# raznem/spp-rl

Hardware: AMD Instinct MI355X
Metric: env-steps/sec (rollout+update) SPP-SAC Hopper-v2 (higher is better)
Workload: dtype fp32

## Files before the change

### spp-rl_amd/csrc/api.hip

```cpp
#include <dlfcn.h>
#include <stdarg.h>
#include <stdio.h>
#include <string.h>

#include <algorithm>
#include <memory>
#include <string>
#include <vector>

#include "../../include/spprl.h"
#include "internal.h"
#include "replay.h"
#include "sac_kernels.h"

#include "optim.hip"
#include "ppo.hip"
#include "replay.hip"
#include "stats.hip"
#include "sac.hip"
#include "ddpg.hip"
#include "kset.h"
#ifdef SPP_SINGLE_TU
#include "ks_dw.hip"
#include "ks_sac_hopper.hip"
// ... 507 lines not shown
      else
        hipLaunchKernelGGL(k_st_bracket<kStSampSmall / 1024>, dim3(ob), dim3(1024), 0, st, (const uint32_t*)samp, S,
                           h->sf_bounds, Sl, (int64_t)ob * Sl, 5);
      h->bounds_dp1 = true;
      h->sf_gen = ~0ull;
    }
    StPassArgs pa{h->d, len, h->sf_bounds, pivot, h->sf_part, h->sf_cpart, h->sf_wgl, h->sf_wgn, h->sf_ovf,
                  h->sf_ovf_n, cap, ovf_cap};
    st_launch_pass(pa, nblk, st);
    hipLaunchKernelGGL(k_dp_reduce, dim3(ob, 2), dim3(kStSelThreads), 0, st, ob, nblk, cap, ovf_cap,
                       (const double*)h->sf_part,
                       (const uint32_t*)h->sf_cpart, (const uint32_t*)h->sf_wgl, (const uint32_t*)h->sf_wgn,
                       (const uint32_t*)h->sf_ovf, (const uint32_t*)h->sf_ovf_n, exch, h->dp_cand, dp_ncand);
  } else if (phase <= 5) {
    hipLaunchKernelGGL(k_dp_round, dim3(ob, 2), dim3(kStSelThreads), 0, st, da, phase - 2);
  } else {
    hipLaunchKernelGGL(k_dp_final, dim3(ob, 2), dim3(128), 0, st, da);
  }
  SPP_CHECK_HIP(hipGetLastError());
  return SPP_OK;
}

int sppReplayObsStatsDPHistSize(sppReplayHandle h) {
  if (!h) return -1;
  const int ob = h->d.ob;
  return std::max(ob, std::min(ob, 32) * 4) * 256;
}

sppStatus sppReplayObsStatsDP(sppReplayHandle h, int step, const float* pivot, double* sums, uint32_t* hist,
                              int64_t n_global, float* mean, float* std, float* max_obs, float* min_obs,
                              int first_update, int* done, void* stream) {
  SPP_REQUIRE(h && pivot && sums && hist && mean && std && max_obs && min_obs && done && step >= 0,
              SPP_E_INVALID_ARG, "obs_stats_dp: bad args");
  const int ob = h->d.ob;
  SPP_REQUIRE(ob <= 16 * kStatsColsPerThread, SPP_E_SHAPE, "obs_stats_dp: ob %d > %d", ob, 16 * kStatsColsPerThread);
  SPP_REQUIRE(n_global > 10 && n_global < ((int64_t)1 << 31), SPP_E_INVALID_ARG, "obs_stats_dp: n_global %lld",
              (long long)n_global);
  sppStatus s = stats_alloc(h);
  if (s) return s;
  hipStream_t st = S(stream);
  const int npass = stats_npass(h);
  SPP_REQUIRE(step <= npass + 1, SPP_E_INVALID_ARG, "obs_stats_dp: step %d > %d", step, npass + 1);
  *done = 0;
  if (step == 0) {
    SPP_CHECK_HIP(hipMemsetAsync(hist, 0, sizeof(uint32_t) * sppReplayObsStatsDPHistSize(h), st));
    if (h->len > 0) {
      stats_pass1(h, hist, pivot, st);
      hipLaunchKernelGGL(k_stats_reduce_part, dim3(ob), dim3(256), 0, st, (const double*)h->st_part, kStatsBlocks,
                         ob, sums);
    } else {
      SPP_CHECK_HIP(hipMemsetAsync(sums, 0, sizeof(double) * ob * 2, st));
    }
  } else {
    if (step == 1) {
      hipLaunchKernelGGL(k_stats_sel, dim3(ob), dim3(256), 0, st, hist, 1, ob, 0, ob, 24, 8, 1, (const double*)sums,
                         n_global, h->st_state, h->st_mean, max_obs, min_obs, first_update);
      hipLaunchKernelGGL(k_stats_moments_out, dim3(1), dim3(128), 0, st, h->d, (const double*)h->st_mean, mean, std,
                         pivot);
    } else {
      stats_sel(h, step - 2, hist, n_global, max_obs, min_obs, first_update, st);
    }
    if (step - 1 < npass) {
      if (h->len > 0) stats_pk(h, step - 1, hist, st);
    } else {
      *done = 1;
    }
  }
  SPP_CHECK_HIP(hipGetLastError());
  return SPP_OK;
}

sppStatus sppGaeScan(const float* rew, const float* v, const float* v_next, const uint8_t* done,
                     const uint8_t* end, int64_t T, int64_t E, double gamma, double lam, int mode, float* q_out,
                     float* adv, void* stream) {
  SPP_REQUIRE(T >= 0 && E > 0 && mode >= -1 && mode <= 1, SPP_E_INVALID_ARG, "gae: T=%lld E=%lld mode=%d",
              (long long)T, (long long)E, mode);
  if (T == 0) return SPP_OK;
  SPP_REQUIRE(rew && v && v_next && done && end && adv, SPP_E_INVALID_ARG, "gae: null input");
  if (mode < 0) mode = E >= 64 ? 0 : 1;
  const double disc = lam * gamma;
  if (mode == 0)
    hipLaunchKernelGGL(k_gae_seq, dim3(cdiv(E, 256)), dim3(256), 0, S(stream), rew, v, v_next, done, end, T, E,
                       (float)gamma, disc, q_out, adv);
  else
    hipLaunchKernelGGL(k_gae_scan, dim3(E), dim3(kScanThreads), 0, S(stream), rew, v, v_next, done, end, T, E,
                       (float)gamma, (float)disc, q_out, adv);
  SPP_CHECK_HIP(hipGetLastError());
  return SPP_OK;
}

sppStatus sppPpoClipLoss(const float* lp_old, const float* lp_new, const float* adv, int B, float eps, float* grad,
                         float* out2, void* stream) {
  SPP_REQUIRE(lp_old && lp_new && adv && out2 && B > 0, SPP_E_INVALID_ARG, "clip loss: bad args");
  const int nblk = cdiv(B, 256);
  double* part = nullptr;
  SPP_CHECK_HIP(hipMallocAsync((void**)&part, sizeof(double) * 2 * nblk, S(stream)));
  hipLaunchKernelGGL(k_ppo_clip, dim3(nblk), dim3(256), 0, S(stream), lp_old, lp_new, adv, B, eps, grad, part);
  hipLaunchKernelGGL(k_ppo_clip_finish, dim3(1), dim3(256), 0, S(stream), (const double*)part, nblk, B, out2);
  SPP_CHECK_HIP(hipFreeAsync(part, S(stream)));
  SPP_CHECK_HIP(hipGetLastError());
  return SPP_OK;
}

sppStatus sppAdvNormalize(const float* adv, int64_t n, float* out, void* stream) {
  SPP_REQUIRE(adv && out && n > 0, SPP_E_INVALID_ARG, "adv normalize: bad args");
  const int nblk = (int)std::min<int64_t>(cdiv(n, 256), 1024);
  double* part = nullptr;
  SPP_CHECK_HIP(hipMallocAsync((void**)&part, sizeof(double) * 2 * nblk, S(stream)));
  hipLaunchKernelGGL(k_adv_moments, dim3(nblk), dim3(256), 0, S(stream), adv, n, part);
  hipLaunchKernelGGL(k_adv_norm, dim3(nblk), dim3(256), 0, S(stream), adv, n, (const double*)part, nblk, out);
  SPP_CHECK_HIP(hipFreeAsync(part, S(stream)));
  SPP_CHECK_HIP(hipGetLastError());
  return SPP_OK;
}

sppStatus sppAdvSums(const float* adv, int64_t n, double* sums2, void* stream) {
  SPP_REQUIRE(adv && sums2 && n >= 0, SPP_E_INVALID_ARG, "adv sums: bad args");
  if (n == 0) {
    SPP_CHECK_HIP(hipMemsetAsync(sums2, 0, sizeof(double) * 2, S(stream)));
    return SPP_OK;
  }
  const int nblk = (int)std::min<int64_t>(cdiv(n, 256), 1024);
  double* part = nullptr;
  SPP_CHECK_HIP(hipMallocAsync((void**)&part, sizeof(double) * 2 * nblk, S(stream)));
  hipLaunchKernelGGL(k_adv_moments, dim3(nblk), dim3(256), 0, S(stream), adv, n, part);
  hipLaunchKernelGGL(k_adv_sum2, dim3(1), dim3(64), 0, S(stream), (const double*)part, nblk, sums2);
  SPP_CHECK_HIP(hipFreeAsync(part, S(stream)));
  SPP_CHECK_HIP(hipGetLastError());
  return SPP_OK;
}

sppStatus sppAdvNormalizeGlobal(const float* adv, int64_t n_local, const double* sums2, int64_t n_global, float* out,
                                void* stream) {
  SPP_REQUIRE(adv && out && sums2 && n_local >= 0 && n_global > 0, SPP_E_INVALID_ARG, "adv normalize dp: bad args");
  if (n_local == 0) return SPP_OK;
  hipLaunchKernelGGL(k_adv_norm_g, dim3((int)std::min<int64_t>(cdiv(n_local, 256), 1024)), dim3(256), 0, S(stream),
                     adv, n_local, sums2, n_global, out);
  SPP_CHECK_HIP(hipGetLastError());
  return SPP_OK;
}

sppStatus sppSynthEnvStep(const float* A, const float* obs, const float* action, int E, int ob, int ac,
                          float* next_obs, float* reward, void* stream) {
  SPP_REQUIRE(A && obs && action && next_obs && reward && E > 0, SPP_E_INVALID_ARG, "synth env: bad args");
  hipLaunchKernelGGL(k_synth_env, dim3(cdiv((int64_t)E * ob, 256)), dim3(256), 0, S(stream), A, obs, action, E, ob, ac, next_obs,
                     reward);
  SPP_CHECK_HIP(hipGetLastError());
  return SPP_OK;
}


sppStatus sppRandUniform(float* out, int64_t n, const float* lo, const float* hi, int period, uint64_t seed,
                         uint64_t offset, void* stream) {
  SPP_REQUIRE((out || n == 0) && lo && hi && period > 0, SPP_E_INVALID_ARG, "rand uniform: bad args");
  if (n == 0) return SPP_OK;
  hipLaunchKernelGGL(k_rand_uniform, dim3(cdiv((n + 3) / 4, 256)), dim3(256), 0, S(stream), out, n, lo, hi, period,
                     seed, offset);
  SPP_CHECK_HIP(hipGetLastError());
  return SPP_OK;
}

sppStatus sppEpisodeAccum(const float* rew, const uint8_t* end, int E, float* ep_ret, double* sums, void* stream) {
  SPP_REQUIRE(rew && ep_ret && sums && E > 0, SPP_E_INVALID_ARG, "episode accum: bad args");
  hipLaunchKernelGGL(k_episode_accum, dim3(cdiv(E, 256)), dim3(256), 0, S(stream), rew, end, E, ep_ret, sums);
  SPP_CHECK_HIP(hipGetLastError());
  return SPP_OK;
}

sppStatus sppSynthEnvReset(float* obs, const uint8_t* mask, int E, int ob, uint64_t seed, uint64_t offset,
                           void* stream) {
  SPP_REQUIRE(obs && E > 0 && ob > 0, SPP_E_INVALID_ARG, "synth reset: bad args");
  hipLaunchKernelGGL(k_synth_reset, dim3(cdiv((int64_t)E * ob, 256)), dim3(256), 0, S(stream), obs, mask, E, ob, seed,
                     offset);
  SPP_CHECK_HIP(hipGetLastError());
  return SPP_OK;
}

sppStatus sppObsNormalize(const float* x, int64_t rows, int ob, const float* lo, const float* hi, const float* mean,
                          const float* std, int min_max, int inverse, float* out, void* stream) {
  SPP_REQUIRE(x && out && rows >= 0 && ob > 0, SPP_E_INVALID_ARG, "normalize: bad args");
  SPP_REQUIRE(min_max ? (lo && hi) : (mean && std), SPP_E_INVALID_ARG, "normalize: missing statistics");
  if (rows == 0) return SPP_OK;
  const int64_t n = rows * ob;
  hipLaunchKernelGGL(k_obs_normalize, dim3(cdiv(n, 256)), dim3(256), 0, S(stream), x, n, ob, lo, hi, mean, std,
                     min_max, inverse, out);
  SPP_CHECK_HIP(hipGetLastError());
  return SPP_OK;
}
}

namespace spp {

struct NetBufs {
  float *p = nullptr, *g = nullptr, *m = nullptr, *v = nullptr;
  int64_t n = 0;
};

template <typename T>
struct DevArray {
  T* ptr = nullptr;
  size_t n = 0;
  hipError_t alloc(size_t count) {
    n = count;
    return hipMalloc(&ptr, sizeof(T) * std::max<size_t>(count, 1));
  }
  void release() {
    if (ptr) hipFree(ptr);
    ptr = nullptr;
  }
};

struct DwSet {
  DevArray<float> slab;
  DevArray<DwJob> jobs;
  DevArray<int> items;
  int B = -1;
  int j0[2] = {0, 0}, nj[2] = {0, 0}, ioff[2] = {0, 0}, nitems[2] = {0, 0};
  int nlds[2] = {0, 0};
  int64_t max_elems[2] = {1, 1};
  bool bf16 = false;
  void release() { slab.release(); jobs.release(); items.release(); }
};

static bool find_kset(int algo, int ob, int aout, int ac, bool acmc, bool bf16, KernelSet* ks) {
  if (bf16) {
#if !defined(SPP_ONLY_HOPPER) || defined(SPP_ONLY_BF16)
    return algo == SPP_ALGO_SAC_ACM && kset_sac_bf16(ob, aout, ac, acmc, ks);
#else
    return false;
#endif
  }
  if (algo == SPP_ALGO_SAC) {
#ifndef SPP_ONLY_HOPPER
    return kset_sac_vanilla(ob, aout, ac, acmc, ks);
#else
    return false;
#endif
  }
  if (algo == SPP_ALGO_DDPG) {
#ifndef SPP_ONLY_HOPPER
    return kset_ddpg_vanilla(ob, aout, ac, acmc, ks);
#else
    return false;
#endif
  }
  if (algo == SPP_ALGO_SAC_ACM) {
    if (kset_sac_hopper(ob, aout, ac, acmc, ks)) return true;
#if defined(SPP_ONLY_HOPPER) && defined(SPP_WITH_HCHEETAH)
    if (kset_sac_hcheetah(ob, aout, ac, acmc, ks)) return true;
#endif
#ifndef SPP_ONLY_HOPPER
    if (kset_sac_hcheetah(ob, aout, ac, acmc, ks)) return true;
    if (kset_sac_ant(ob, aout, ac, acmc, ks)) return true;
    if (kset_sac_small(ob, aout, ac, acmc, ks)) return true;
  } else if (algo == SPP_ALGO_DDPG_ACM) {
    if (kset_ddpg(ob, aout, ac, acmc, ks)) return true;
    if (kset_ddpg_ant(ob, aout, ac, acmc, ks)) return true;
#endif
  }
  return false;
}

}

struct sppAgent {
  sppAgentConfig cfg{};
  int device = 0, num_cu = 256;
  bool team_ok = true;
  KernelSet ks{};
  NetBufs net[SPP_NET_COUNT];
  int64_t nsize[SPP_NET_COUNT] = {};
  int cin = 0, Bmax = 0, Bpmax = 0;
  int64_t steps[4] = {0, 0, 0, 0};
  const float *lo = nullptr, *hi = nullptr, *mean = nullptr, *std = nullptr;
  double* alpha_state = nullptr;
  float* alpha_f32 = nullptr;
  DevArray<float> limits;
  DevArray<float4> pk;
  std::vector<PackJob> pj_actor, pj_acm, pj_targ, pj_critic_fwd, pj_critic_all, pj_acmreg;
  bool ddpg = false;
  bool plain = false;
  DevArray<PackJob> d_pj;
  int o_actor = 0, o_acm = 0, o_targ = 0, o_cfwd = 0, o_call = 0, o_acmreg = 0;
  std::vector<TabSeg> tab;
  int tab_floats = 0;
  ActorDev actor{};
  CriticDev critic[2]{}, targ[2]{};
  AcmDev acm{};
  const float4* acm_W1n = nullptr;
  BAcmDev bacm{};
  ActorDev actor_targ{};
  const float4 *bacm_W1n = nullptr, *bacm_W21n = nullptr;
  BAcmScratch bz{};
  float *RBH = nullptr, *RBH1 = nullptr, *RS21 = nullptr, *RBP1 = nullptr, *RPZ = nullptr, *RPZ21 = nullptr;
  DevArray<float> scratch;
  float *S = nullptr, *S2 = nullptr, *ACT = nullptr, *AENV = nullptr, *R = nullptr, *DN = nullptr, *EPS1 = nullptr,
        *EPS2 = nullptr;
  float *H1[2] = {}, *H2[2] = {}, *D1[2] = {}, *D2[2] = {}, *DQ[2] = {};
  float *AH1 = nullptr, *AH2 = nullptr, *AD1 = nullptr, *AD2 = nullptr, *ADH = nullptr;
  float *Z1 = nullptr, *Z2 = nullptr, *T3 = nullptr, *part = nullptr;
  float *aux = nullptr;
  float* GAD = nullptr;
  uint64_t* MASK = nullptr;
  float *RX = nullptr, *RZ1 = nullptr, *RZ2 = nullptr, *RP1 = nullptr, *RP2 = nullptr, *RP3 = nullptr;
  DwSet dws[2];
  DevArray<AdamJob> d_adam;
  int cur_B = -1;
  float* w3p[2] = {};
  int64_t w3p_stride = 0;
  float* alpha_grad = nullptr;
  DevArray<float> sgd_slab;
  DevArray<int> sgd_sync;
  int sgd_max_wg = -1;
  bool timing = false;
  std::vector<hipEvent_t> tev[5];
  size_t tused[5] = {0, 0, 0, 0, 0};
};

static void tmark(sppAgent* a, int kind, hipStream_t st) {
  if (!a->timing) return;
  auto& v = a->tev[kind];
  if (a->tused[kind] == v.size()) {
    hipEvent_t e;
    hipEventCreate(&e);
    v.push_back(e);
  }
  hipEventRecord(v[a->tused[kind]++], st);
}

namespace spp {

static int64_t sac_actor_size(int ob, int aout) { return 256LL * ob + 256 + 65536 + 256 + 2LL * (aout * 256 + aout); }
static int64_t critic_size(int cin) { return 256LL * cin + 256 + 65536 + 256 + 256 + 1; }
static int64_t acm_size(int in, int ac) { return 64LL * in + 64 + 32 * 64 + 32 + (int64_t)ac * 32 + ac; }
static int64_t ddpg_actor_size(int ob, int aout) { return 256LL * ob + 256 + 65536 + 256 + (int64_t)aout * 256 + aout; }
static int64_t bacm_size(int in, int ac) {
  return 1 + ac + 100LL * in + 100 + 50 * 100 + 50 + 50LL * in + 50 + (int64_t)ac * 50 + ac;
}

static MapDesc nat(int n) { return MapDesc{MAP_NAT, n, 0, 0, 0}; }
static MapDesc cat(int n0, int n1) { return MapDesc{MAP_CAT, n0, blocks_of(n0), n1, n0}; }
static MapDesc pair(int n) { return MapDesc{MAP_PAIR, n, 0, 0, 0}; }

}

static sppStatus build_packs(sppAgent* a) {
  const int ob = a->cfg.ob, aout = a->cfg.aout, ac = a->cfg.ac;
  const int ca = a->cfg.acm_critic ? ac : aout;
  const int cin = ob + ca;
  for (int k = 0; k < SPP_NET_COUNT; ++k) {
    const bool used = a->ddpg ? (k == SPP_NET_ACTOR || k == SPP_NET_CRITIC1 || k == SPP_NET_CRITIC1_TARG ||
                                 (k == SPP_NET_ACM && !a->plain) || k == SPP_NET_ACTOR_TARG)
                              : k != SPP_NET_ACTOR_TARG;
    SPP_REQUIRE(!used || a->net[k].p, SPP_E_STATE, "network %d parameters not bound", k);
  }
  struct MatSpec {
    std::vector<PackJob>* list;
    PackJob job;
    const float4** slot;
  };
  std::vector<MatSpec> ms;
  auto M = [&](std::vector<PackJob>* list, const float* W, const float* W2, int split, int ld, int trans, int coff,
               MapDesc out, MapDesc in, int NBO, int NBI, const float4** slot, int ib = 0) {
    PackJob j{W, W2, split, ld, trans, coff, out, in, NBO, NBI, ib, nullptr, a->cfg.mlp_bf16 ? 1 : 0};
    ms.push_back({list, j, slot});
  };
  a->tab.clear();
  int toff = 0;
  auto T = [&](const float* v, int n, const float* v2 = nullptr, int n2 = 0) {
    const int off = toff, tot = (int)round_up(n + n2, 32);
    a->tab.push_back(TabSeg{v, n, v2 ? n : tot, off, 0});
    if (v2) a->tab.push_back(TabSeg{v2, n2, tot - n, off + n, 0});
    toff += tot;
    return off;
  };
  if (!a->ddpg) {
    {
      const float* P = a->net[SPP_NET_ACTOR].p;
      const float *W1 = P, *b1 = W1 + 256 * ob, *W2 = b1 + 256, *b2 = W2 + 65536, *Wp = b2 + 256, *bp = Wp + aout * 256,
                  *Ws = bp + aout, *bs = Ws + aout * 256;
      M(&a->pj_actor, W1, nullptr, 1 << 30, ob, 0, 0, nat(256), nat(ob), 8, blocks_of(ob), &a->actor.W1);
      M(&a->pj_actor, W2, nullptr, 1 << 30, 256, 0, 0, nat(256), nat(256), 8, 8, &a->actor.W2, 1);
      M(&a->pj_actor, Wp, Ws, aout, 256, 0, 0, nat(2 * aout), nat(256), blocks_of(2 * aout), 8, &a->actor.Wh, 1);
      M(&a->pj_actor, W2, nullptr, 1 << 30, 256, 1, 0, nat(256), nat(256), 8, 8, &a->actor.W2T, 1);
      M(&a->pj_actor, Wp, Ws, aout, 256, 1, 0, nat(256), pair(aout), 8, (aout + 15) / 16, &a->actor.WhT);
      if (a->cfg.mlp_bf16)
        M(&a->pj_actor, Wp, Ws, aout, 256, 0, 0, pair(aout), nat(256), (aout + 15) / 16, 8, &a->actor.WhP, 1);
      a->actor.tb1 = T(b1, 256);
      a->actor.tb2 = T(b2, 256);
      a->actor.tbh = T(bp, aout, bs, aout);
    }
  } else {
    for (int t = 0; t < 2; ++t) {
      const float* P = a->net[t == 0 ? SPP_NET_ACTOR : SPP_NET_ACTOR_TARG].p;
      ActorDev& ad = t == 0 ? a->actor : a->actor_targ;
      std::vector<PackJob>* l = t == 0 ? &a->pj_actor : &a->pj_targ;
      const float *W1 = P, *b1 = W1 + 256 * ob, *W2 = b1 + 256, *b2 = W2 + 65536, *W3 = b2 + 256, *b3 = W3 + aout * 256;
      M(l, W1, nullptr, 1 << 30, ob, 0, 0, nat(256), nat(ob), 8, blocks_of(ob), &ad.W1);
      M(l, W2, nullptr, 1 << 30, 256, 0, 0, nat(256), nat(256), 8, 8, &ad.W2, 1);
      M(l, W3, nullptr, 1 << 30, 256, 0, 0, nat(aout), nat(256), blocks_of(aout), 8, &ad.Wh, 1);
      if (t == 0) {
        M(l, W2, nullptr, 1 << 30, 256, 1, 0, nat(256), nat(256), 8, 8, &ad.W2T, 1);
        M(l, W3, nullptr, 1 << 30, 256, 1, 0, nat(256), nat(aout), 8, blocks_of(aout), &ad.WhT);
      }
      ad.tb1 = T(b1, 256);
      ad.tb2 = T(b2, 256);
      ad.tbh = T(b3, aout);
    }
  }
  if (!a->ddpg) {
    {
      const float* P = a->net[SPP_NET_ACM].p;
      const int in = 2 * ob;
      const float *W1 = P, *b1 = W1 + 64 * in, *W2 = b1 + 64, *b2 = W2 + 32 * 64, *W3 = b2 + 32, *b3 = W3 + ac * 32;
      M(&a->pj_acm, W1, nullptr, 1 << 30, in, 0, 0, nat(64), cat(ob, aout), 2, blocks_of(ob) + blocks_of(aout),
        &a->acm.W1);
      M(&a->pj_acm, W2, nullptr, 1 << 30, 64, 0, 0, nat(32), nat(64), 1, 2, &a->acm.W2);
      M(&a->pj_acm, W3, nullptr, 1 << 30, 32, 0, 0, nat(ac), nat(32), 1, 1, &a->acm.W3);
      M(&a->pj_acm, W3, nullptr, 1 << 30, 32, 1, 0, nat(32), nat(ac), 1, 1, &a->acm.W3T);
      M(&a->pj_acm, W2, nullptr, 1 << 30, 64, 1, 0, nat(64), nat(32), 2, 1, &a->acm.W2T);
      M(&a->pj_acm, W1, nullptr, 1 << 30, in, 1, ob, nat(aout), nat(64), blocks_of(aout), 2, &a->acm.W1Ta);
      M(&a->pj_acm, W1, nullptr, 1 << 30, in, 0, 0, nat(64), nat(in), 2, blocks_of(in), &a->acm_W1n);
      a->acm.tb1 = T(b1, 64);
      a->acm.tb2 = T(b2, 32);
      a->acm.tb3 = T(b3, ac);
    }
  } else if (!a->plain) {
    const float* P = a->net[SPP_NET_ACM].p;
    const int in = 2 * ob;
    const float *t = P, *t1 = P + 1, *W1 = t1 + ac, *b1 = W1 + 100 * in, *W2 = b1 + 100, *b2 = W2 + 50 * 100,
                *W21 = b2 + 50, *b21 = W21 + 50 * in, *W3 = b21 + 50, *b3 = W3 + ac * 50;
    BAcmDev& B = a->bacm;
    const int nbi = blocks_of(ob) + blocks_of(aout);
    M(&a->pj_acm, W1, nullptr, 1 << 30, in, 0, 0, nat(100), cat(ob, aout), 4, nbi, &B.W1);
    M(&a->pj_acm, W21, nullptr, 1 << 30, in, 0, 0, nat(50), cat(ob, aout), 2, nbi, &B.W21);
    M(&a->pj_acm, W2, nullptr, 1 << 30, 100, 0, 0, nat(50), nat(100), 2, 4, &B.W2);
    M(&a->pj_acm, W3, nullptr, 1 << 30, 50, 0, 0, nat(ac), nat(50), 1, 2, &B.W3);
    M(&a->pj_acm, W3, nullptr, 1 << 30, 50, 1, 0, nat(50), nat(ac), 2, 1, &B.W3T);
    M(&a->pj_acm, W2, nullptr, 1 << 30, 100, 1, 0, nat(100), nat(50), 4, 2, &B.W2T);
    M(&a->pj_acm, W1, nullptr, 1 << 30, in, 1, ob, nat(aout), nat(100), blocks_of(aout), 4, &B.W1Ta);
    M(&a->pj_acm, W21, nullptr, 1 << 30, in, 1, ob, nat(aout), nat(50), blocks_of(aout), 2, &B.W21Ta);
    M(&a->pj_acm, W1, nullptr, 1 << 30, in, 0, 0, nat(100), nat(in), 4, blocks_of(in), &a->bacm_W1n);
    M(&a->pj_acm, W21, nullptr, 1 << 30, in, 0, 0, nat(50), nat(in), 2, blocks_of(in), &a->bacm_W21n);
    B.tb1 = T(b1, 100);
    B.tb21 = T(b21, 50);
    B.tb2 = T(b2, 50);
    B.tb3 = T(b3, ac);
    B.t = t;
    B.t1 = t1;
  }
  for (int t = 0; t < 4; ++t) {
    if (a->ddpg && (t == 1 || t == 3)) continue;
    const int netid = t < 2 ? SPP_NET_CRITIC1 + t : SPP_NET_CRITIC1_TARG + (t - 2);
    CriticDev& cd = t < 2 ? a->critic[t] : a->targ[t - 2];
    const float* P = a->net[netid].p;
    const float *W1 = P, *b1 = W1 + 256 * cin, *W2 = b1 + 256, *b2 = W2 + 65536, *w3 = b2 + 256, *b3 = w3 + 256;
    std::vector<PackJob>* fl = t < 2 ? &a->pj_critic_fwd : &a->pj_targ;
    M(fl, W1, nullptr, 1 << 30, cin, 0, 0, nat(256), cat(ob, ca), 8, blocks_of(ob) + blocks_of(ca), &cd.W1);
    M(fl, W2, nullptr, 1 << 30, 256, 0, 0, nat(256), nat(256), 8, 8, &cd.W2, 1);
    if (t < 2) {
      M(fl, W2, nullptr, 1 << 30, 256, 1, 0, nat(256), nat(256), 8, 8, &cd.W2T, 1);
      M(fl, W1, nullptr, 1 << 30, cin, 1, ob, nat(ca), nat(256), blocks_of(ca), 8, &cd.W1Ta, 1);
    }
    cd.tb1 = T(b1, 256);
    cd.tb2 = T(b2, 256);
    cd.tw3 = T(w3, 256);
    cd.b3 = b3;
  }
  a->tab_floats = toff;
  const int extra = 3 * (int)round_up(aout, 32) + (int)round_up(std::max(ac, 1), 32);
  SPP_REQUIRE(toff + extra <= kTabMax && (int)a->tab.size() + 4 <= kTabSegs, SPP_E_SHAPE,
              "LDS table too large (%d floats, %d segments)", toff + extra, (int)a->tab.size() + 4);
  size_t nf4 = 0;
  for (auto& m : ms) nf4 += (size_t)m.job.NBO * m.job.NBI * 4 * 64;
  a->pk.release();
  SPP_CHECK_HIP(a->pk.alloc(nf4));
  size_t of = 0;
  for (auto& m : ms) {
    m.job.dst = a->pk.ptr + of;
    *m.slot = m.job.dst;
    of += (size_t)m.job.NBO * m.job.NBI * 4 * 64;
    m.list->push_back(m.job);
  }
  a->pj_critic_all = a->pj_critic_fwd;
  std::vector<PackJob> all;
  a->o_actor = (int)all.size(); all.insert(all.end(), a->pj_actor.begin(), a->pj_actor.end());
  a->o_acm = (int)all.size(); all.insert(all.end(), a->pj_acm.begin(), a->pj_acm.end());
  a->o_targ = (int)all.size(); all.insert(all.end(), a->pj_targ.begin(), a->pj_targ.end());
  a->o_cfwd = (int)all.size(); all.insert(all.end(), a->pj_critic_fwd.begin(), a->pj_critic_fwd.end());
  a->d_pj.release();
  SPP_CHECK_HIP(a->d_pj.alloc(all.size()));
  SPP_CHECK_HIP(hipMemcpy(a->d_pj.ptr, all.data(), sizeof(PackJob) * all.size(), hipMemcpyHostToDevice));
  return SPP_OK;
}

static void launch_pack(sppAgent* a, int off, int n, hipStream_t st) {
  if (n > 0) hipLaunchKernelGGL(k_pack_matrix, dim3(64, n), dim3(256), 0, st, (const PackJob*)(a->d_pj.ptr + off));
}

#ifndef SPP_DW_BIG16
#define SPP_DW_BIG16 1
#endif
static sppStatus finalize_dw(DwSet& D, std::vector<DwJob>& jobs, int nph, int Bp, int B, int num_cu) {
  auto is_big = [](const DwJob& j) {
    return (int64_t)round_up(j.N, 32) * round_up(j.K0 + j.K1, 32) >= 128 * 128;
  };
  auto lds_big = [Bp](const DwJob& j) {
    return Bp >= 8192 && j.N == 256 && j.K0 == 256 && j.K1 == 0 &&
           (!j.bf16 || (SPP_DW_BIG16 && j.a_bf && j.x_bf && Bp % 64 == 0));
  };
  auto assign_splits = [&](int first, int count) {
    double big[2] = {0.0, 0.0};
    for (int i = first; i < first + count; ++i)
      if (!jobs[i].fused && is_big(jobs[i]))
        big[lds_big(jobs[i]) ? 0 : 1] += (double)round_up(jobs[i].N, 32) * round_up(jobs[i].K0 + jobs[i].K1, 32);
    for (int i = first; i < first + count; ++i) {
      DwJob& j = jobs[i];
      if (j.fused) continue;
      const double pm = (double)round_up(j.N, 32) * round_up(j.K0 + j.K1, 32);
      const bool thin_n = j.N <= 128, thin_k = j.K0 + j.K1 <= 128;
      j.wsplit = thin_n && thin_k ? 4 : (thin_n != thin_k ? 2 : 1);
      int ns = is_big(j) ? (int)std::lround(num_cu * pm / big[lds_big(j) ? 0 : 1])
                         : std::min(cdiv(Bp, 2048), std::max(1, 256 / j.wsplit));
      if (!is_big(j)) ns = std::max(ns, std::min(cdiv(Bp, 32 * j.wsplit), 4));
      ns = std::max(1, std::min(ns, std::max(1, Bp / 32)));
      j.split_len = (int)round_up(cdiv(Bp, ns), lds_big(j) && j.bf16 ? 64 : 32 * j.wsplit);
      j.nsplit = cdiv(Bp, j.split_len);
    }
  };
  for (int ph = 0; ph < nph; ++ph) assign_splits(D.j0[ph], D.nj[ph]);
  size_t need = 0;
  for (int ph = 0; ph < nph; ++ph) {
    size_t off = 0;
    for (int j = D.j0[ph]; j < D.j0[ph] + D.nj[ph]; ++j) {
      if (jobs[j].nsplit * jobs[j].wsplit > 1) {
        jobs[j].slab = nullptr;
        off += (size_t)jobs[j].nsplit * jobs[j].wsplit * jobs[j].slab_stride;
      }
    }
    need = std::max(need, off);
  }
  if (need > D.slab.n) {
    D.slab.release();
    SPP_CHECK_HIP(D.slab.alloc(need));
  }
  std::vector<int> items;
  for (int ph = 0; ph < nph; ++ph) {
    size_t off = 0;
    std::vector<int> jj, ss;
    for (int j = D.j0[ph]; j < D.j0[ph] + D.nj[ph]; ++j) {
      if (jobs[j].nsplit * jobs[j].wsplit > 1) {
        jobs[j].slab = D.slab.ptr + off;
        off += (size_t)jobs[j].nsplit * jobs[j].wsplit * jobs[j].slab_stride;
      }
    }
    D.nlds[ph] = 0;
    for (int pass = 0; pass < 3; ++pass)
      for (int j = D.j0[ph]; j < D.j0[ph] + D.nj[ph]; ++j) {
        const int cls = lds_big(jobs[j]) ? 0 : (is_big(jobs[j]) ? 1 : 2);
        if (cls != pass || jobs[j].fused) continue;
        for (int sp = 0; sp < jobs[j].nsplit; ++sp) {
          jj.push_back(j - D.j0[ph]);
          ss.push_back(sp);
          if (pass == 0) ++D.nlds[ph];
        }
      }
    D.max_elems[ph] = 1;
    for (int j = D.j0[ph]; j < D.j0[ph] + D.nj[ph]; ++j) {
      const int64_t el = (int64_t)jobs[j].N * (jobs[j].K0 + jobs[j].K1) + jobs[j].N;
      D.max_elems[ph] = std::max<int64_t>(D.max_elems[ph], el * dw_red_group(jobs[j].nsplit * jobs[j].wsplit, el));
    }
    D.ioff[ph] = (int)items.size();
    D.nitems[ph] = (int)jj.size();
    items.insert(items.end(), jj.begin(), jj.end());
    items.insert(items.end(), ss.begin(), ss.end());
  }
  D.jobs.release();
  D.items.release();
  SPP_CHECK_HIP(D.jobs.alloc(jobs.size()));
  SPP_CHECK_HIP(D.items.alloc(items.size()));
  SPP_CHECK_HIP(hipMemcpy(D.jobs.ptr, jobs.data(), sizeof(DwJob) * jobs.size(), hipMemcpyHostToDevice));
  SPP_CHECK_HIP(hipMemcpy(D.items.ptr, items.data(), sizeof(int) * items.size(), hipMemcpyHostToDevice));
  D.B = B;
  D.bf16 = !jobs.empty() && jobs[0].bf16;
  for (const DwJob& j : jobs)
    if ((j.bf16 != 0) != D.bf16) return SPP_E_STATE;
  return SPP_OK;
}

static int phase_grid(sppAgent* a, int Bp);
static int sac_grid(sppAgent* a, int Bp);
static int sac_critic_grid(sppAgent* a, int Bp);
static bool sac_team(sppAgent* a, int Bp);
static bool ddpg_team(sppAgent* a, int Bp);
static int ddpg_grid(sppAgent* a, int Bp);
static sppStatus build_dw(sppAgent* a, int set, int B) {
  const int Bp = (int)round_up(B, 32);
  const int ob = a->cfg.ob, aout = a->cfg.aout, ac = a->cfg.ac;
  const int ca = a->cfg.acm_critic ? ac : aout, cin = ob + ca;
  std::vector<DwJob> jobs;
  std::vector<const float*> b16;
  if (a->cfg.mlp_bf16 && !a->ddpg && set == 0)
    b16 = {a->H1[0], a->H1[1], a->H2[0], a->H2[1], a->D1[0], a->D1[1], a->D2[0], a->D2[1],
           a->AH1, a->AH2, a->AD1, a->AD2};
  auto is16 = [&](const float* p) { return p && std::find(b16.begin(), b16.end(), p) != b16.end(); };
  auto J = [&](const float* A, int N, const float* X0, int K0, const float* X1, int K1, float* dW, float* db,
               int nrow2 = -1, float* dW2 = nullptr, float* db2 = nullptr) {
    DwJob j{};
    j.A = A; j.N = N; j.X0 = X0; j.K0 = K0; j.X1 = X1; j.K1 = K1; j.dW = dW; j.db = db; j.Bp = Bp;
    j.nrow2 = nrow2 < 0 ? N : nrow2;
    j.dW2 = dW2; j.db2 = db2;
    j.slab_stride = round_up((int64_t)N * (K0 + K1) + N, 4);
    j.bf16 = a->cfg.mlp_bf16 ? 1 : 0;
    j.a_bf = is16(A) ? 1 : 0;
    j.x_bf = is16(X0) ? 1 : 0;
    jobs.push_back(j);
  };
  DwSet& D = a->dws[set];
  int nph = 0;
  if (a->ddpg) {
    if (set == 0) {
      float* G = a->net[SPP_NET_CRITIC1].g;
      float *gW1 = G, *gb1 = gW1 + 256 * cin, *gW2 = gb1 + 256, *gb2 = gW2 + 65536, *gw3 = gb2 + 256, *gb3 = gw3 + 256;
      J(a->D1[0], 256, a->S, ob, a->cfg.acm_critic ? a->AENV : a->ACT, ca, gW1, gb1);
      J(a->D2[0], 256, a->H1[0], 256, nullptr, 0, gW2, gb2);
      int fused0 = -1;
      if (ob <= 32) {
        J(nullptr, 1, nullptr, 256, nullptr, 0, gw3, gb3);
        jobs.back().fused = 1;
        jobs.back().nsplit = ddpg_grid(a, Bp) * (ddpg_team(a, Bp) ? kTeamDCritic : kWavesPerWG);
        jobs.back().wsplit = 1;
        fused0 = (int)jobs.size() - 1;
      } else {
        J(a->DQ[0], 1, a->H2[0], 256, nullptr, 0, gw3, gb3);
      }
      D.j0[0] = 0;
      D.nj[0] = (int)jobs.size();
      float* A = a->net[SPP_NET_ACTOR].g;
      float *aW1 = A, *ab1 = aW1 + 256 * ob, *aW2 = ab1 + 256, *ab2 = aW2 + 65536, *aW3 = ab2 + 256,
            *ab3 = aW3 + aout * 256;
      J(a->AD1, 256, a->S, ob, nullptr, 0, aW1, ab1);
      J(a->AD2, 256, a->AH1, 256, nullptr, 0, aW2, ab2);
      J(a->ADH, aout, a->AH2, 256, nullptr, 0, aW3, ab3);
      D.j0[1] = D.nj[0];
      D.nj[1] = (int)jobs.size() - D.nj[0];
      nph = 2;
      sppStatus s = finalize_dw(D, jobs, nph, Bp, B, a->num_cu);
      a->w3p[0] = a->w3p[1] = fused0 >= 0 ? jobs[fused0].slab : nullptr;
      a->w3p_stride = fused0 >= 0 ? jobs[fused0].slab_stride : 0;
      return s;
    } else {
      SPP_REQUIRE(!a->plain, SPP_E_STATE, "vanilla DDPG has no ACM to regress");
      float* G = a->net[SPP_NET_ACM].g;
      const int in = 2 * ob;
      float *gW1 = G + 1 + ac, *gb1 = gW1 + 100 * in, *gW2 = gb1 + 100, *gb2 = gW2 + 50 * 100, *gW21 = gb2 + 50,
            *gb21 = gW21 + 50 * in, *gW3 = gb21 + 50, *gb3 = gW3 + ac * 50;
      J(a->RBP1, 100, a->RX, in, nullptr, 0, gW1, gb1);
      J(a->RPZ, 50, a->RBH, 100, nullptr, 0, gW2, gb2);
      J(a->RPZ21, 50, a->RX, in, nullptr, 0, gW21, gb21);
      J(a->RP3, ac, a->RBH1, 50, nullptr, 0, gW3, gb3);
      D.j0[0] = 0;
      D.nj[0] = (int)jobs.size();
      nph = 1;
    }
  } else if (set == 0) {
    const bool fuse3 = !a->cfg.mlp_bf16 || SPP_BF16_FUSE3;
    int fused_idx[2] = {-1, -1};
    for (int i = 0; i < 2; ++i) {
      float* G = a->net[SPP_NET_CRITIC1 + i].g;
      float *gW1 = G, *gb1 = gW1 + 256 * cin, *gW2 = gb1 + 256, *gb2 = gW2 + 65536, *gw3 = gb2 + 256, *gb3 = gw3 + 256;
      J(a->D1[i], 256, a->S, ob, a->cfg.acm_critic ? a->AENV : a->ACT, ca, gW1, gb1);
      J(a->D2[i], 256, a->H1[i], 256, nullptr, 0, gW2, gb2);
      if (!fuse3) {
        J(a->DQ[i], 1, a->H2[i], 256, nullptr, 0, gw3, gb3);
        continue;
      }
      J(nullptr, 1, nullptr, 256, nullptr, 0, gw3, gb3);
      jobs.back().fused = 1;
      jobs.back().nsplit = sac_critic_grid(a, Bp) * (sac_team(a, Bp) ? kTeamCritic : kWavesPerWG);
      jobs.back().wsplit = 1;
      fused_idx[i] = (int)jobs.size() - 1;
    }
    D.j0[0] = 0;
    D.nj[0] = (int)jobs.size();
    float* G = a->net[SPP_NET_ACTOR].g;
    float *gW1 = G, *gb1 = gW1 + 256 * ob, *gW2 = gb1 + 256, *gb2 = gW2 + 65536, *gWp = gb2 + 256,
          *gbp = gWp + aout * 256, *gWs = gbp + aout, *gbs = gWs + aout * 256;
    J(a->AD1, 256, a->S, ob, nullptr, 0, gW1, gb1);
    J(a->AD2, 256, a->AH1, 256, nullptr, 0, gW2, gb2);
    J(a->ADH, 2 * aout, a->AH2, 256, nullptr, 0, gWp, gbp, aout, gWs, gbs);
    D.j0[1] = D.nj[0];
    D.nj[1] = (int)jobs.size() - D.nj[0];
    nph = 2;
    sppStatus s = finalize_dw(D, jobs, nph, Bp, B, a->num_cu);
    for (int i = 0; i < 2; ++i) a->w3p[i] = fuse3 ? jobs[fused_idx[i]].slab : nullptr;
    a->w3p_stride = fuse3 ? jobs[fused_idx[0]].slab_stride : 0;
    return s;
  } else {
    float* G = a->net[SPP_NET_ACM].g;
    const int in = 2 * ob;
    float *gW1 = G, *gb1 = gW1 + 64 * in, *gW2 = gb1 + 64, *gb2 = gW2 + 32 * 64, *gW3 = gb2 + 32, *gb3 = gW3 + ac * 32;
    J(a->RP1, 64, a->RX, in, nullptr, 0, gW1, gb1);
    J(a->RP2, 32, a->RZ1, 64, nullptr, 0, gW2, gb2);
    J(a->RP3, ac, a->RZ2, 32, nullptr, 0, gW3, gb3);
    D.j0[0] = 0;
    D.nj[0] = (int)jobs.size();
    nph = 1;
  }
  return finalize_dw(D, jobs, nph, Bp, B, a->num_cu);
}


static void launch_dw_set(DwSet& D, int ph, hipStream_t st) {
  const int* ij = D.items.ptr + D.ioff[ph];
  const int* is = ij + D.nitems[ph];
  const DwJob* jobs = D.jobs.ptr + D.j0[ph];
  launch_dw_kernels(jobs, ij, is, D.nitems[ph], D.nlds[ph], D.nj[ph], D.max_elems[ph], D.bf16, st);
}
static void launch_dw(sppAgent* a, int set, int ph, hipStream_t st) { launch_dw_set(a->dws[set], ph, st); }

static sppStatus build_adam(sppAgent* a) {
  AdamJob jobs[4] = {};
  for (int i = 0; i < (a->ddpg ? 1 : 2); ++i) {
    NetBufs& n = a->net[SPP_NET_CRITIC1 + i];
    jobs[i] = AdamJob{n.p, n.g, n.m, n.v, a->net[SPP_NET_CRITIC1_TARG + i].p, n.n};
  }
  NetBufs& na = a->net[SPP_NET_ACTOR];
  jobs[2] = AdamJob{na.p, na.g, na.m, na.v, a->ddpg ? a->net[SPP_NET_ACTOR_TARG].p : nullptr, na.n};
  NetBufs& nm = a->net[SPP_NET_ACM];
  jobs[3] = AdamJob{nm.p, nm.g, nm.m, nm.v, nullptr, nm.n};
  if (!a->d_adam.ptr) SPP_CHECK_HIP(a->d_adam.alloc(4));
  SPP_CHECK_HIP(hipMemcpy(a->d_adam.ptr, jobs, sizeof(jobs), hipMemcpyHostToDevice));
  return SPP_OK;
}

static void launch_adam(sppAgent* a, int first, int count, int64_t n, int64_t step, float lr, float tau,
                        hipStream_t st) {
  const double bc1 = 1.0 - std::pow(0.9, (double)step), bc2s = std::sqrt(1.0 - std::pow(0.999, (double)step));
  hipLaunchKernelGGL(k_adam, dim3(std::max(1, std::min(cdiv(n, 256 * 4), 1024)), count), dim3(256), 0, st,
                     (const AdamJob*)(a->d_adam.ptr + first), (float)(-(lr / bc1)), (float)bc2s, tau);
}

static SacArgs make_args(sppAgent* a, int B) {
  SacArgs p{};
  p.B = B;
  p.Bp = (int)round_up(B, 32);
  p.inv_B = 1.f / (float)B;
  p.S = a->S; p.S2 = a->S2; p.ACT = a->ACT; p.AENV = a->AENV; p.R = a->R; p.DN = a->DN;
  p.EPS1 = a->EPS1; p.EPS2 = a->EPS2;
  p.min_max = a->cfg.min_max_denormalize;
  p.lo = a->lo; p.hi = a->hi; p.mean = a->mean; p.std = a->std;
  p.actor_lim = a->limits.ptr;
  p.acm_lim = a->limits.ptr + a->cfg.aout;
  p.gamma = a->cfg.gamma;
  p.custom_loss = a->cfg.custom_loss;
  p.norm_closs = a->cfg.norm_closs;
  p.alpha = a->alpha_f32;
  p.actor = a->actor;
  for (int i = 0; i < 2; ++i) {
    p.critic[i] = a->critic[i];
    p.targ[i] = a->targ[i];
    p.H1[i] = a->H1[i]; p.H2[i] = a->H2[i]; p.D1[i] = a->D1[i]; p.D2[i] = a->D2[i]; p.DQ[i] = a->DQ[i];
    p.W3P[i] = a->w3p[i];
  }
  p.w3p_stride = a->w3p_stride;
  p.acm = a->acm;
  p.bacm = a->bacm;
  p.actor_targ = a->actor_targ;
  p.AH1 = a->AH1; p.AH2 = a->AH2; p.AD1 = a->AD1; p.AD2 = a->AD2; p.ADH = a->ADH;
  p.part = a->part;
  p.nseg = (int)a->tab.size();
  for (int i = 0; i < p.nseg; ++i) p.seg[i] = a->tab[i];
  int off = a->tab_floats;
  auto X = [&](const float* v, int n) {
    const int o = off, np = (int)round_up(std::max(n, 1), 32);
    p.seg[p.nseg++] = TabSeg{v ? v : a->limits.ptr, v ? n : 0, np, o, 0};
    off += np;
    return o;
  };
  const int aout = a->cfg.aout;
  p.t_lim = X(a->limits.ptr, aout);
  p.t_alim = X(a->limits.ptr + aout, a->cfg.ac);
  p.t_n0 = X(p.min_max ? a->lo : a->mean, aout);
  p.t_n1 = X(p.min_max ? a->hi : a->std, aout);
  return p;
}

static int phase_grid(sppAgent* a, int Bp) {
  const int ntiles = Bp / 32;
  return std::max(1, std::min(cdiv(ntiles, kWavesPerWG), a->num_cu));
}
static bool sac_team(sppAgent* a, int Bp) {
  return a->ks.critic_team && a->ks.actor_team && a->team_ok && Bp / 32 <= a->num_cu;
}
static int sac_grid(sppAgent* a, int Bp) {
  return sac_team(a, Bp) ? std::max(1, std::min(Bp / 32, a->num_cu)) : phase_grid(a, Bp);
}
static int sac_critic_grid(sppAgent* a, int Bp) {
  const int nt = std::max(1, Bp / 32);
  return sac_team(a, Bp) && 2 * nt <= a->num_cu ? 2 * nt : sac_grid(a, Bp);
}

static bool ddpg_team(sppAgent* a, int Bp) {
  return a->ks.dcritic_team && a->ks.dactor_team && a->team_ok && Bp / 32 <= a->num_cu;
}
static int ddpg_grid(sppAgent* a, int Bp) {
  return ddpg_team(a, Bp) ? std::max(1, std::min(Bp / 32, a->num_cu)) : phase_grid(a, Bp);
}

static sppStatus check_ready(sppAgent* a) {
  SPP_REQUIRE(a->ddpg || (a->alpha_state && a->alpha_f32), SPP_E_STATE, "alpha not bound");
  SPP_REQUIRE(a->cfg.min_max_denormalize ? (a->lo && a->hi) : (a->mean && a->std), SPP_E_STATE,
              "normalizer not bound");
  SPP_REQUIRE(a->limits.ptr, SPP_E_STATE, "limits not set");
  if (!a->pk.ptr) {
    sppStatus s = build_packs(a);
    if (s) return s;
    if ((s = build_adam(a))) return s;
    a->dws[0].B = a->dws[1].B = -1;
  }
  return SPP_OK;
}

extern "C" {

sppStatus sppAgentCreate(sppAgentHandle* out, const sppAgentConfig* cfg, int device) {
  SPP_REQUIRE(out && cfg, SPP_E_INVALID_ARG, "null arg");
  SPP_REQUIRE(cfg->algo == SPP_ALGO_SAC_ACM || cfg->algo == SPP_ALGO_DDPG_ACM || cfg->algo == SPP_ALGO_SAC ||
                  cfg->algo == SPP_ALGO_DDPG,
              SPP_E_INVALID_ARG, "unsupported algo %d", cfg->algo);
  SPP_REQUIRE(cfg->algo != SPP_ALGO_SAC || (cfg->acm_critic == 0 && cfg->aout == cfg->ac && cfg->custom_loss == 0.f),
              SPP_E_INVALID_ARG, "vanilla SAC: the actor emits the env action (aout == ac), no ACM critic / loss");
  SPP_REQUIRE(cfg->algo != SPP_ALGO_DDPG || (cfg->acm_critic == 0 && cfg->aout == cfg->ac && cfg->custom_loss == 0.f),
              SPP_E_INVALID_ARG, "vanilla DDPG: the actor emits the env action (aout == ac), no ACM critic / loss");
  SPP_REQUIRE(cfg->algo != SPP_ALGO_DDPG || cfg->mlp_bf16 == 0, SPP_E_INVALID_ARG, "vanilla DDPG: fp32 only");
  SPP_REQUIRE(cfg->max_batch > 0, SPP_E_INVALID_ARG, "max_batch must be > 0");
  KernelSet ks;
  SPP_REQUIRE(find_kset(cfg->algo, cfg->ob, cfg->aout, cfg->ac, cfg->acm_critic != 0, cfg->mlp_bf16 != 0, &ks),
              SPP_E_SHAPE, "no kernel instantiation for algo %d (ob=%d, aout=%d, ac=%d, bf16=%d)", cfg->algo, cfg->ob,
              cfg->aout, cfg->ac, cfg->mlp_bf16);
  SPP_CHECK_HIP(hipSetDevice(device));
  auto a = std::make_unique<sppAgent>();
  a->cfg = *cfg;
  a->device = device;
  a->ks = ks;
  hipDeviceProp_t prop;
  SPP_CHECK_HIP(hipGetDeviceProperties(&prop, device));
  a->num_cu = prop.multiProcessorCount;
  {
    const char* t = getenv("SPP_SAC_TEAM");
    a->team_ok = !(t && t[0] == '0');
  }
  const int ob = cfg->ob, aout = cfg->aout, ac = cfg->ac;
  a->cin = ob + (cfg->acm_critic ? ac : aout);
  a->ddpg = cfg->algo == SPP_ALGO_DDPG_ACM || cfg->algo == SPP_ALGO_DDPG;
  a->plain = cfg->algo == SPP_ALGO_SAC || cfg->algo == SPP_ALGO_DDPG;
  const bool dd = a->ddpg;
  a->nsize[SPP_NET_ACTOR] = dd ? ddpg_actor_size(ob, aout) : sac_actor_size(ob, aout);
  a->nsize[SPP_NET_ACTOR_TARG] = dd ? ddpg_actor_size(ob, aout) : 0;
  a->nsize[SPP_NET_CRITIC1] = a->nsize[SPP_NET_CRITIC1_TARG] = critic_size(a->cin);
  a->nsize[SPP_NET_CRITIC2] = a->nsize[SPP_NET_CRITIC2_TARG] = dd ? 0 : critic_size(a->cin);
  a->nsize[SPP_NET_ACM] = dd ? (a->plain ? 0 : bacm_size(2 * ob, ac)) : acm_size(2 * ob, ac);
  a->Bmax = cfg->max_batch;
  const int64_t Bp = round_up(cfg->max_batch, 32);
  SPP_REQUIRE((int64_t)Bp * 256 * 4 < ((int64_t)1 << 31), SPP_E_SHAPE, "max_batch %d too large (31-bit buffer offsets)",
              cfg->max_batch);
  a->Bpmax = (int)Bp;
  const int64_t ntiles = Bp / 32;
  const int64_t per = Bp;
  int64_t total = 0;
  auto take = [&](int64_t rows) { int64_t o = total; total += rows * per; return o; };
  const int64_t oS = take(ob), oS2 = take(ob), oACT = take(aout), oAENV = take(ac), oR = take(1), oDN = take(1),
                oE1 = take(aout), oE2 = take(aout);
  int64_t oH1[2] = {}, oH2[2] = {}, oD1[2] = {}, oD2[2] = {}, oDQ[2] = {};
  for (int i = 0; i < (dd ? 1 : 2); ++i) {
    oH1[i] = take(256); oH2[i] = take(256); oD1[i] = take(256); oD2[i] = take(256); oDQ[i] = take(1);
  }
  const int64_t oAH1 = take(256), oAH2 = take(256), oAD1 = take(256), oAD2 = take(256), oADH = take(2 * aout);
  const int64_t oZ1 = take(dd ? 128 : 64), oZ2 = take(dd ? 64 : 32), oT3 = take(ac);
  const int64_t oRX = take(2 * ob), oRZ1 = take(dd ? 128 : 64), oRZ2 = take(dd ? 64 : 32), oRP1 = take(dd ? 128 : 64),
                oRP2 = take(dd ? 64 : 32), oRP3 = take(ac);
  const int64_t oRS21 = dd ? take(64) : 0, oRPZ21 = dd ? take(64) : 0;
  const int64_t oGAD = take(aout), oMASK = take(16);
  const int64_t oPart = total;
  total += ntiles * kBParts + 64;
  const int64_t oAux = total;
  total += 16;
  hipError_t e = a->scratch.alloc(total);
  if (e != hipSuccess) {
    set_error("scratch alloc %.2f GB: %s", total * 4.0 / 1e9, hipGetErrorString(e));
    return SPP_E_OOM;
  }
  SPP_CHECK_HIP(hipMemset(a->scratch.ptr, 0, sizeof(float) * total));
  float* b = a->scratch.ptr;
  a->S = b + oS; a->S2 = b + oS2; a->ACT = b + oACT; a->AENV = b + oAENV; a->R = b + oR; a->DN = b + oDN;
  a->EPS1 = b + oE1; a->EPS2 = b + oE2;
  for (int i = 0; i < 2; ++i) {
    a->H1[i] = b + oH1[i]; a->H2[i] = b + oH2[i]; a->D1[i] = b + oD1[i]; a->D2[i] = b + oD2[i]; a->DQ[i] = b + oDQ[i];
  }
  a->AH1 = b + oAH1; a->AH2 = b + oAH2; a->AD1 = b + oAD1; a->AD2 = b + oAD2; a->ADH = b + oADH;
  a->Z1 = b + oZ1; a->Z2 = b + oZ2; a->T3 = b + oT3;
  a->GAD = b + oGAD;
  a->MASK = reinterpret_cast<uint64_t*>(b + oMASK);
  a->RX = b + oRX; a->RZ1 = b + oRZ1; a->RZ2 = b + oRZ2; a->RP1 = b + oRP1; a->RP2 = b + oRP2; a->RP3 = b + oRP3;
  if (dd) {
    a->bz = BAcmScratch{a->Z1, a->Z2, a->T3};
    a->RBH = a->RZ1; a->RBH1 = a->RZ2; a->RBP1 = a->RP1; a->RPZ = a->RP2;
    a->RS21 = b + oRS21; a->RPZ21 = b + oRPZ21;
  }
  a->part = b + oPart;
  a->aux = b + oAux;
  SPP_CHECK_HIP(a->limits.alloc(aout + ac));
  *out = a.release();
  return SPP_OK;
}

sppStatus sppAgentDestroy(sppAgentHandle a) {
  if (!a) return SPP_OK;
  hipSetDevice(a->device);
  hipDeviceSynchronize();
  a->limits.release(); a->pk.release(); a->d_pj.release();
  for (auto& v : a->tev)
    for (auto e : v) hipEventDestroy(e);
  a->scratch.release(); a->d_adam.release();
  for (auto& D : a->dws) D.release();
  delete a;
  return SPP_OK;
}

sppStatus sppAgentNetSize(sppAgentHandle a, int net, int64_t* n) {
  SPP_REQUIRE(a && n && net >= 0 && net < SPP_NET_COUNT, SPP_E_INVALID_ARG, "bad net id");
  *n = a->nsize[net];
  return SPP_OK;
}

sppStatus sppAgentBindNet(sppAgentHandle a, int net, float* p, float* g, float* m, float* v) {
  SPP_REQUIRE(a && net >= 0 && net < SPP_NET_COUNT && p, SPP_E_INVALID_ARG, "bind: bad args");
  const bool trainable = net == SPP_NET_ACTOR || net == SPP_NET_CRITIC1 || net == SPP_NET_CRITIC2 || net == SPP_NET_ACM;
  SPP_REQUIRE(!trainable || (g && m && v), SPP_E_INVALID_ARG, "bind: trainable net %d needs grad/m/v", net);
  const bool changed = a->net[net].p != p || a->net[net].g != g;
  a->net[net] = NetBufs{p, g, m, v, a->nsize[net]};
  if (changed) {
    a->pk.release();
    a->pj_actor.clear(); a->pj_acm.clear(); a->pj_targ.clear(); a->pj_critic_fwd.clear(); a->pj_critic_all.clear();
    a->tab.clear();
  }
  return SPP_OK;
}

sppStatus sppAgentSetLimits(sppAgentHandle a, const float* actor_lim, const float* acm_lim) {
  SPP_REQUIRE(a && actor_lim && acm_lim, SPP_E_INVALID_ARG, "null");
  SPP_CHECK_HIP(hipMemcpy(a->limits.ptr, actor_lim, sizeof(float) * a->cfg.aout, hipMemcpyHostToDevice));
  SPP_CHECK_HIP(hipMemcpy(a->limits.ptr + a->cfg.aout, acm_lim, sizeof(float) * a->cfg.ac, hipMemcpyHostToDevice));
  return SPP_OK;
}

sppStatus sppAgentBindNormalizer(sppAgentHandle a, const float* lo, const float* hi, const float* mean,
                                 const float* std) {
  SPP_REQUIRE(a, SPP_E_INVALID_ARG, "null");
  a->lo = lo; a->hi = hi; a->mean = mean; a->std = std;
  return SPP_OK;
}

sppStatus sppAgentBindAlpha(sppAgentHandle a, double* st, float* af) {
  SPP_REQUIRE(a && st && af, SPP_E_INVALID_ARG, "null");
  a->alpha_state = st;
  a->alpha_f32 = af;
  return SPP_OK;
}

sppStatus sppAgentSetLr(sppAgentHandle a, float actor_lr, float critic_lr, float alpha_lr, float acm_lr) {
  SPP_REQUIRE(a, SPP_E_INVALID_ARG, "null handle");
  if (actor_lr >= 0.f) a->cfg.actor_lr = actor_lr;
  if (critic_lr >= 0.f) a->cfg.critic_lr = critic_lr;
  if (alpha_lr >= 0.f) a->cfg.alpha_lr = alpha_lr;
  if (acm_lr >= 0.f) a->cfg.acm_lr = acm_lr;
  return SPP_OK;
}
sppStatus sppAgentSetSteps(sppAgentHandle a, int64_t s0, int64_t s1, int64_t s2, int64_t s3) {
  SPP_REQUIRE(a, SPP_E_INVALID_ARG, "null");
  a->steps[0] = s0; a->steps[1] = s1; a->steps[2] = s2; a->steps[3] = s3;
  return SPP_OK;
}
sppStatus sppAgentGetSteps(sppAgentHandle a, int64_t* s) {
  SPP_REQUIRE(a && s, SPP_E_INVALID_ARG, "null");
  for (int i = 0; i < 4; ++i) s[i] = a->steps[i];
  return SPP_OK;
}

static sppStatus stage(sppAgentHandle a, const sppBatch* bt, const float* e1, const float* e2, hipStream_t st) {
  SPP_REQUIRE(bt && bt->B > 0 && bt->B <= a->Bmax, SPP_E_SHAPE, "batch B=%d outside (0, max_batch=%d]",
              bt ? bt->B : -1, a->Bmax);
  SPP_REQUIRE(bt->obs && bt->next_obs && bt->reward && bt->done && bt->acm_action, SPP_E_INVALID_ARG,
              "batch: null field");
  SPP_REQUIRE(a->cfg.acm_critic || bt->action, SPP_E_INVALID_ARG, "batch.action required without acm_critic");
  StageArgs s{};
  s.B = bt->B; s.Bp = (int)round_up(bt->B, 32); s.ob = a->cfg.ob; s.aout = a->cfg.aout; s.ac = a->cfg.ac;
  s.obs = bt->obs; s.next_obs = bt->next_obs; s.act = bt->action; s.rew = bt->reward; s.acm = bt->acm_action;
  s.done = bt->done; s.eps1 = e1; s.eps2 = e2;
  s.S = a->S; s.S2 = a->S2; s.ACT = a->ACT; s.AENV = a->AENV; s.R = a->R; s.DN = a->DN; s.EPS1 = a->EPS1;
  s.EPS2 = a->EPS2;
  hipLaunchKernelGGL(k_stage_batch, dim3(cdiv(s.Bp, 256)), dim3(256), 0, st, s);
  a->cur_B = bt->B;
  return SPP_OK;
}

static sppStatus critic_grads_staged(sppAgentHandle a, float* losses, hipStream_t st) {
  SPP_REQUIRE(!a->ddpg, SPP_E_STATE, "not a SAC_AcM agent");
  const int B = a->cur_B;
  SPP_REQUIRE(B > 0, SPP_E_STATE, "no staged batch");
  sppStatus s = check_ready(a);
  if (s) return s;
  if (a->dws[0].B != B) {
    s = build_dw(a, 0, B);
    if (s) return s;
  }
  launch_pack(a, a->o_actor, (int)(a->pj_actor.size() + a->pj_acm.size() + a->pj_targ.size() + a->pj_critic_fwd.size()),
              st);
  SacArgs p = make_args(a, B);
  const int grid = sac_critic_grid(a, p.Bp);
  tmark(a, 0, st);
  const bool team = sac_team(a, p.Bp);
  hipLaunchKernelGGL(team ? a->ks.critic_team : a->ks.critic, dim3(grid), dim3(team ? 64 * kTeamCritic : 256), 0, st, p);
  tmark(a, 0, st);
  SPP_CHECK_HIP(hipGetLastError());
  tmark(a, 2, st);
  launch_dw(a, 0, 0, st);
  tmark(a, 2, st);
  hipLaunchKernelGGL(k_finalize_critic, dim3(1), dim3(kFinThreads), 0, st, (const float*)a->part, p.Bp / 32, B, losses);
  SPP_CHECK_HIP(hipGetLastError());
  return SPP_OK;
}

sppStatus sppSacAcmCriticGrads(sppAgentHandle a, const sppBatch* bt, const float* eps_next, float* losses,
                               void* stream) {
  SPP_REQUIRE(a, SPP_E_INVALID_ARG, "null");
  if (bt) {
    sppStatus s = stage(a, bt, eps_next, nullptr, S(stream));
    if (s) return s;
  } else if (eps_next) {
    const int Bp = (int)round_up(a->cur_B, 32);
    SPP_REQUIRE(a->cur_B > 0, SPP_E_STATE, "no staged batch");
    hipLaunchKernelGGL(k_eps_copy_fm, dim3(cdiv((int64_t)a->cfg.aout * Bp, 256)), dim3(256), 0, S(stream), eps_next,
                       a->EPS1, a->cfg.aout, a->cur_B, Bp);
  }
  return critic_grads_staged(a, losses, S(stream));
}

sppStatus sppSacAcmCriticApply(sppAgentHandle a, void* stream) {
  SPP_REQUIRE(a && a->d_adam.ptr, SPP_E_STATE, "agent not ready");
  a->steps[1] += 1;
  tmark(a, 3, S(stream));
  launch_adam(a, 0, 2, a->net[SPP_NET_CRITIC1].n, a->steps[1], a->cfg.critic_lr, a->cfg.tau, S(stream));
  tmark(a, 3, S(stream));
  SPP_CHECK_HIP(hipGetLastError());
  return SPP_OK;
}

static sppStatus actor_grads(sppAgentHandle a, float* losses, hipStream_t st) {
  SPP_REQUIRE(!a->ddpg, SPP_E_STATE, "not a SAC_AcM agent");
  const int B = a->cur_B;
  SPP_REQUIRE(B > 0, SPP_E_STATE, "no staged batch");
  launch_pack(a, a->o_cfwd, (int)a->pj_critic_fwd.size(), st);
  SacArgs p = make_args(a, B);
  AcmScratch z{a->Z1, a->Z2, a->T3, a->GAD, a->MASK};
  const int grid = sac_grid(a, p.Bp);
  tmark(a, 1, st);
  const bool team = sac_team(a, p.Bp);
  hipLaunchKernelGGL(team ? a->ks.actor_team : a->ks.actor, dim3(grid), dim3(team ? 64 * kTeamActor : 256), 0, st, p, z);
  if (a->ks.actor_heads) hipLaunchKernelGGL(a->ks.actor_heads, dim3(grid), dim3(256), 0, st, p, z);
  tmark(a, 1, st);
  SPP_CHECK_HIP(hipGetLastError());
  tmark(a, 2, st);
  launch_dw(a, 0, 1, st);
  tmark(a, 2, st);
  hipLaunchKernelGGL(k_actor_partials, dim3(1), dim3(kFinThreads), 0, st, (const float*)a->part, p.Bp / 32, B, a->cfg.aout,
                     a->cfg.custom_loss, (double)a->cfg.target_entropy, a->alpha_grad ? a->alpha_grad : a->aux,
                     losses);
  SPP_CHECK_HIP(hipGetLastError());
  return SPP_OK;
}

sppStatus sppSacAcmActorGrads(sppAgentHandle a, const float* eps_cur, float* losses, void* stream) {
  SPP_REQUIRE(a, SPP_E_INVALID_ARG, "null");
  const int B = a->cur_B;
  SPP_REQUIRE(B > 0, SPP_E_STATE, "no staged batch");
  const int Bp = (int)round_up(B, 32);
  if (eps_cur)
    hipLaunchKernelGGL(k_eps_copy_fm, dim3(cdiv((int64_t)a->cfg.aout * Bp, 256)), dim3(256), 0, S(stream), eps_cur,
                       a->EPS2, a->cfg.aout, B, Bp);
  return actor_grads(a, losses, S(stream));
}

sppStatus sppAgentBindAlphaGrad(sppAgentHandle a, float* g) {
  SPP_REQUIRE(a, SPP_E_INVALID_ARG, "null");
  a->alpha_grad = g;
  return SPP_OK;
}

sppStatus sppSacAcmDrawEps(sppAgentHandle a, uint64_t seed, uint64_t counter, void* stream) {
  SPP_REQUIRE(a && a->cur_B > 0, SPP_E_STATE, "no staged batch");
  const int B = a->cur_B, Bp = (int)round_up(B, 32);
  SPP_REQUIRE((int64_t)a->cfg.aout * Bp < ((int64_t)1 << 31), SPP_E_SHAPE, "draw_eps: aout * Bp >= 2^31");
  const int64_t quads = (int64_t)a->cfg.aout * Bp / 4;
  hipLaunchKernelGGL(k_eps_fm, dim3(cdiv(quads, 256), 2), dim3(256), 0, S(stream), a->EPS1, a->cfg.aout, B, Bp, seed,
                     2 * counter, a->EPS2, 2 * counter + 1);
  SPP_CHECK_HIP(hipGetLastError());
  return SPP_OK;
}

sppStatus sppAgentReadEps(sppAgentHandle a, int which, float* out, void* stream) {
  SPP_REQUIRE(a && out && (which == 0 || which == 1), SPP_E_INVALID_ARG, "read_eps: bad args");
  SPP_REQUIRE(a->cur_B > 0, SPP_E_STATE, "no staged batch");
  const int B = a->cur_B, Bp = (int)round_up(B, 32);
  hipLaunchKernelGGL(k_eps_read_fm, dim3(cdiv((int64_t)a->cfg.aout * B, 256)), dim3(256), 0, S(stream),
                     (const float*)(which ? a->EPS2 : a->EPS1), out, a->cfg.aout, B, Bp);
  SPP_CHECK_HIP(hipGetLastError());
  return SPP_OK;
}

static std::vector<PackJob> images_of(sppAgent* a, int net) {
  std::vector<PackJob> out;
  const NetBufs& nb = a->net[net];
  if (!nb.p) return out;
  for (auto* l : {&a->pj_actor, &a->pj_acm, &a->pj_targ, &a->pj_critic_fwd})
    for (const PackJob& j : *l)
      if (j.W >= nb.p && j.W < nb.p + nb.n) out.push_back(j);
  return out;
}

sppStatus sppAgentImageCount(sppAgentHandle a, int net, int* n) {
  SPP_REQUIRE(a && n && net >= 0 && net < SPP_NET_COUNT, SPP_E_INVALID_ARG, "image_count: bad args");
  *n = (int)images_of(a, net).size();
  return SPP_OK;
}

sppStatus sppAgentUnpackImage(sppAgentHandle a, int net, int i, float* out, void* stream) {
  SPP_REQUIRE(a && out && net >= 0 && net < SPP_NET_COUNT, SPP_E_INVALID_ARG, "unpack_image: bad args");
  const std::vector<PackJob> js = images_of(a, net);
  SPP_REQUIRE(i >= 0 && i < (int)js.size(), SPP_E_INVALID_ARG, "unpack_image: image %d of %d", i, (int)js.size());
  hipLaunchKernelGGL(k_unpack_matrix, dim3(64), dim3(256), 0, S(stream), js[i], (const float*)a->net[net].p, out);
  SPP_CHECK_HIP(hipGetLastError());
  return SPP_OK;
}

sppStatus sppAgentSetTiming(sppAgentHandle a, int enable) {
  SPP_REQUIRE(a, SPP_E_INVALID_ARG, "null");
  a->timing = enable != 0;
  return SPP_OK;
}

sppStatus sppAgentGetTiming(sppAgentHandle a, double* ms, int64_t* cnt) {
  SPP_REQUIRE(a && ms && cnt, SPP_E_INVALID_ARG, "null");
  for (int k = 0; k < 5; ++k) {
    double t = 0.0;
    for (size_t i = 0; i + 1 < a->tused[k]; i += 2) {
      SPP_CHECK_HIP(hipEventSynchronize(a->tev[k][i + 1]));
      float e = 0.f;
      SPP_CHECK_HIP(hipEventElapsedTime(&e, a->tev[k][i], a->tev[k][i + 1]));
      t += e;
    }
    ms[k] = t;
    cnt[k] = (int64_t)(a->tused[k] / 2);
    a->tused[k] = 0;
  }
  return SPP_OK;
}

static sppStatus actor_apply(sppAgentHandle a, float* losses, hipStream_t st) {
  a->steps[0] += 1;
  a->steps[2] += 1;
  tmark(a, 3, st);
  launch_adam(a, 2, 1, a->net[SPP_NET_ACTOR].n, a->steps[0], a->cfg.actor_lr, 0.f, st);
  tmark(a, 3, st);
  hipLaunchKernelGGL(k_alpha_step, dim3(1), dim3(64), 0, st, (const float*)(a->alpha_grad ? a->alpha_grad : a->aux),
                     (double)a->cfg.alpha_lr, a->steps[2], a->alpha_state, a->alpha_f32, losses);
  SPP_CHECK_HIP(hipGetLastError());
  return SPP_OK;
}

sppStatus sppSacAcmActorApply(sppAgentHandle a, float* losses, void* stream) {
  SPP_REQUIRE(a, SPP_E_INVALID_ARG, "null");
  return actor_apply(a, losses, S(stream));
}

sppStatus sppSacAcmUpdate(sppAgentHandle a, const sppBatch* bt, const float* eps_next, const float* eps_cur,
                          float* losses, void* stream) {
  SPP_REQUIRE(a && !a->ddpg, SPP_E_STATE, "not a SAC_AcM agent");
  SPP_REQUIRE(a && eps_next && eps_cur, SPP_E_INVALID_ARG, "eps required (use sppSacAcmUpdateStaged for device draws)");
  hipStream_t st = S(stream);
  sppStatus s = stage(a, bt, eps_next, eps_cur, st);
  if (s) return s;
  if ((s = critic_grads_staged(a, losses, st))) return s;
  if ((s = sppSacAcmCriticApply(a, stream))) return s;
  if ((s = actor_grads(a, losses, st))) return s;
  return actor_apply(a, losses, st);
}

sppStatus sppDdpgAcmCriticGrads(sppAgentHandle a, const sppBatch* bt, float* losses, void* stream) {
  SPP_REQUIRE(a && a->ddpg, SPP_E_STATE, "not a DDPG_AcM agent");
  hipStream_t st = S(stream);
  sppStatus s;
  if (bt && (s = stage(a, bt, nullptr, nullptr, st))) return s;
  const int B = a->cur_B;
  SPP_REQUIRE(B > 0, SPP_E_STATE, "no staged batch");
  if ((s = check_ready(a))) return s;
  if (a->dws[0].B != B && (s = build_dw(a, 0, B))) return s;
  launch_pack(a, a->o_actor, (int)(a->pj_actor.size() + a->pj_acm.size() + a->pj_targ.size() + a->pj_critic_fwd.size()),
              st);
  SacArgs p = make_args(a, B);
  tmark(a, 0, st);
  const bool team = ddpg_team(a, p.Bp);
  hipLaunchKernelGGL(team ? a->ks.dcritic_team : a->ks.dcritic, dim3(ddpg_grid(a, p.Bp)),
                     dim3(team ? 64 * kTeamDCritic : 256), 0, st, p, a->bz);
  tmark(a, 0, st);
  SPP_CHECK_HIP(hipGetLastError());
  tmark(a, 2, st);
  launch_dw(a, 0, 0, st);
  tmark(a, 2, st);
  hipLaunchKernelGGL(k_finalize_ddpg_critic, dim3(1), dim3(kFinThreads), 0, st, (const float*)a->part, p.Bp / 32, B, losses);
  SPP_CHECK_HIP(hipGetLastError());
  return SPP_OK;
}

sppStatus sppDdpgAcmCriticApply(sppAgentHandle a, void* stream) {
  SPP_REQUIRE(a && a->ddpg && a->d_adam.ptr, SPP_E_STATE, "DDPG_AcM agent not ready");
  a->steps[1] += 1;
  tmark(a, 3, S(stream));
  launch_adam(a, 0, 1, a->net[SPP_NET_CRITIC1].n, a->steps[1], a->cfg.critic_lr, a->cfg.tau, S(stream));
  tmark(a, 3, S(stream));
  SPP_CHECK_HIP(hipGetLastError());
  return SPP_OK;
}

sppStatus sppDdpgAcmActorGrads(sppAgentHandle a, float* losses, void* stream) {
  SPP_REQUIRE(a && a->ddpg && a->cur_B > 0, SPP_E_STATE, "DDPG_AcM agent: no staged batch");
  hipStream_t st = S(stream);
  const int B = a->cur_B;
  launch_pack(a, a->o_cfwd, (int)a->pj_critic_fwd.size(), st);
  SacArgs p = make_args(a, B);
  tmark(a, 1, st);
  const bool team = ddpg_team(a, p.Bp);
  hipLaunchKernelGGL(team ? a->ks.dactor_team : a->ks.dactor, dim3(ddpg_grid(a, p.Bp)),
                     dim3(team ? 64 * kTeamDActor : 256), 0, st, p, a->bz);
  tmark(a, 1, st);
  SPP_CHECK_HIP(hipGetLastError());
  tmark(a, 2, st);
  launch_dw(a, 0, 1, st);
  tmark(a, 2, st);
  hipLaunchKernelGGL(k_finalize_ddpg_actor, dim3(1), dim3(kFinThreads), 0, st, (const float*)a->part, p.Bp / 32, B,
                     a->cfg.aout, a->cfg.custom_loss, losses);
  SPP_CHECK_HIP(hipGetLastError());
  return SPP_OK;
}

sppStatus sppDdpgAcmActorApply(sppAgentHandle a, void* stream) {
  SPP_REQUIRE(a && a->ddpg && a->d_adam.ptr, SPP_E_STATE, "DDPG_AcM agent not ready");
  a->steps[0] += 1;
  tmark(a, 3, S(stream));
  launch_adam(a, 2, 1, a->net[SPP_NET_ACTOR].n, a->steps[0], a->cfg.actor_lr, a->cfg.tau, S(stream));
  tmark(a, 3, S(stream));
  SPP_CHECK_HIP(hipGetLastError());
  return SPP_OK;
}

sppStatus sppDdpgAcmUpdate(sppAgentHandle a, const sppBatch* bt, float* losses, void* stream) {
  sppStatus s;
  if ((s = sppDdpgAcmCriticGrads(a, bt, losses, stream))) return s;
  if ((s = sppDdpgAcmCriticApply(a, stream))) return s;
  if ((s = sppDdpgAcmActorGrads(a, losses, stream))) return s;
  return sppDdpgAcmActorApply(a, stream);
}

sppStatus sppAgentStageFromReplay(sppAgentHandle a, sppReplayHandle r, const int64_t* idx, int B, void* stream) {
  SPP_REQUIRE(a && r && idx && B > 0 && B <= a->Bmax, SPP_E_INVALID_ARG, "stage_from_replay: bad args");
  SPP_REQUIRE(r->d.ob == a->cfg.ob && r->d.ac == a->cfg.ac && r->d.aout == a->cfg.aout, SPP_E_SHAPE, "dims differ");
  const int Bp = (int)round_up(B, 32);
  float* act = a->cfg.acm_critic ? nullptr : a->ACT;
  if (r->d.ob > 64)
    hipLaunchKernelGGL(k_replay_stage_fm2, dim3(cdiv(Bp, kStage2Tile)), dim3(256),
                       stage2_lds_bytes(r->d.ob, r->d.aout, r->d.ac, act != nullptr), S(stream), r->d, idx, B, Bp,
                       a->S, a->S2, act, a->AENV, a->R, a->DN);
  else
    hipLaunchKernelGGL(k_replay_stage_fm, dim3(cdiv(Bp, kStageTile)), dim3(256),
                       sizeof(float) * kStageTile * std::max(r->d.ob, r->d.aout), S(stream), r->d, idx, B, Bp, a->S,
                       a->S2, act, a->AENV, a->R, a->DN);
  SPP_CHECK_HIP(hipGetLastError());
  a->cur_B = B;
  return SPP_OK;
}

sppStatus sppAgentStagePost(sppAgentHandle a, int normalize, int act_from_next_obs, void* stream) {
  SPP_REQUIRE(a && a->cur_B > 0, SPP_E_STATE, "stage_post: no staged batch");
  if (!normalize && !act_from_next_obs) return SPP_OK;
  SPP_REQUIRE(!act_from_next_obs || (!a->cfg.acm_critic && a->cfg.aout == a->cfg.ob && a->ACT), SPP_E_INVALID_ARG,
              "stage_post: action = next_obs needs a critic on (obs, actor output) with aout == ob");
  SPP_REQUIRE(normalize >= 0 && normalize <= 2, SPP_E_INVALID_ARG, "stage_post: normalize %d", normalize);
  const int mm = normalize == 2 ? 0 : a->cfg.min_max_denormalize;
  SPP_REQUIRE(!normalize || (mm ? (a->lo && a->hi) : (a->mean && a->std)), SPP_E_STATE,
              "stage_post: normalizer not bound");
  const int B = a->cur_B, Bp = (int)round_up(B, 32), ob = a->cfg.ob;
  hipLaunchKernelGGL(k_stage_post, dim3(cdiv((int64_t)ob * B, 256)), dim3(256), 0, S(stream), a->S, a->S2, a->ACT, ob,
                     B, Bp, a->lo, a->hi, a->mean, a->std, mm, normalize != 0, act_from_next_obs);
  SPP_CHECK_HIP(hipGetLastError());
  return SPP_OK;
}

sppStatus sppSacAcmUpdateStaged(sppAgentHandle a, uint64_t seed, uint64_t counter, float* losses, void* stream) {
  SPP_REQUIRE(a && a->cur_B > 0, SPP_E_STATE, "no staged batch");
  hipStream_t st = S(stream);
  sppStatus s = sppSacAcmDrawEps(a, seed, counter, stream);
  if (s) return s;
  if ((s = critic_grads_staged(a, losses, st))) return s;
  if ((s = sppSacAcmCriticApply(a, stream))) return s;
  if ((s = actor_grads(a, losses, st))) return s;
  return actor_apply(a, losses, st);
}

sppStatus sppAcmRegressGrads(sppAgentHandle a, const float* x, const float* y, int B, float* loss, void* stream) {
  SPP_REQUIRE(a && x && y && B > 0 && B <= a->Bmax, SPP_E_INVALID_ARG, "acm step: bad args (B=%d, max %d)", B,
              a->Bmax);
  SPP_REQUIRE(!(a->ddpg && a->plain), SPP_E_STATE, "vanilla DDPG has no ACM to regress");
  hipStream_t st = S(stream);
  sppStatus s = check_ready(a);
  if (s) return s;
  if (a->dws[1].B != B) {
    if ((s = build_dw(a, 1, B))) return s;
  }
  launch_pack(a, a->o_acm, (int)a->pj_acm.size(), st);
  SacArgs p = make_args(a, B);
  if (a->ddpg) {
    p.bacm.W1 = a->bacm_W1n;
    p.bacm.W21 = a->bacm_W21n;
    BAcmRegArgs g{};
    g.B = B; g.Bp = (int)round_up(B, 32); g.x = x; g.y = y;
    g.XT = a->RX; g.H = a->RBH; g.H1 = a->RBH1; g.S21 = a->RS21; g.P1 = a->RBP1; g.PZ = a->RPZ; g.PZ21 = a->RPZ21;
    g.P3 = a->RP3; g.part = a->part;
    tmark(a, 4, st);
    hipLaunchKernelGGL(a->ks.dreg, dim3(phase_grid(a, g.Bp)), dim3(256), 0, st, p, g);
    SPP_CHECK_HIP(hipGetLastError());
    launch_dw(a, 1, 0, st);
    tmark(a, 4, st);
    hipLaunchKernelGGL(k_finalize_bacm, dim3(1), dim3(256), 0, st, (const float*)a->part, g.Bp / 32, kBParts, B,
                       a->cfg.ac, a->net[SPP_NET_ACM].g, loss);
    SPP_CHECK_HIP(hipGetLastError());
    return SPP_OK;
  }
  p.acm.W1 = a->acm_W1n;
  AcmRegArgs g{};
  g.B = B; g.Bp = (int)round_up(B, 32); g.x = x; g.y = y;
  g.XT = a->RX; g.Z1 = a->RZ1; g.Z2 = a->RZ2; g.P1 = a->RP1; g.P2 = a->RP2; g.P3 = a->RP3; g.part = a->part;
  tmark(a, 4, st);
  hipLaunchKernelGGL(a->ks.acmreg, dim3(phase_grid(a, g.Bp)), dim3(256), 0, st, p, g);
  SPP_CHECK_HIP(hipGetLastError());
  launch_dw(a, 1, 0, st);
  tmark(a, 4, st);
  hipLaunchKernelGGL(k_finalize_acm, dim3(1), dim3(256), 0, st, (const float*)a->part, g.Bp / 32, B, a->cfg.ac, loss);
  SPP_CHECK_HIP(hipGetLastError());
  return SPP_OK;
}

sppStatus sppAcmRegressApply(sppAgentHandle a, void* stream) {
  SPP_REQUIRE(a && a->d_adam.ptr, SPP_E_STATE, "agent not ready");
  SPP_REQUIRE(!(a->ddpg && a->plain), SPP_E_STATE, "vanilla DDPG has no ACM to regress");
  a->steps[3] += 1;
  launch_adam(a, 3, 1, a->net[SPP_NET_ACM].n, a->steps[3], a->cfg.acm_lr, 0.f, S(stream));
  SPP_CHECK_HIP(hipGetLastError());
  return SPP_OK;
}

extern "C++" {
template <int IN, int H2, int OUT, int HEAD, int WV = 4>
static int mlp_sgd_max_wg(int num_cu) {
// ... 902 lines not shown
```

### spp-rl_amd/csrc/kset.h

```cpp
#pragma once
#include "sac.hip"
#include "sac_bf.h"
#include "ddpg.hip"
#include "sac_team.h"
#include "ddpg_team.h"

namespace spp {

struct KernelSet {
  void (*critic)(SacArgs);
  void (*actor)(SacArgs, AcmScratch);
  void (*actor_heads)(SacArgs, AcmScratch);
  void (*act)(SacArgs, ActArgs);
  void (*acmreg)(SacArgs, AcmRegArgs);
  void (*dcritic)(SacArgs, BAcmScratch);
  void (*dactor)(SacArgs, BAcmScratch);
  void (*dact)(SacArgs, ActArgs, BAcmScratch);
  void (*dreg)(SacArgs, BAcmRegArgs);
  void (*critic_team)(SacArgs);
  void (*actor_team)(SacArgs, AcmScratch);
  void (*act_team)(SacArgs, ActArgs);
  void (*dcritic_team)(SacArgs, BAcmScratch);
  void (*dactor_team)(SacArgs, BAcmScratch);
  void (*dact_team)(SacArgs, ActArgs, BAcmScratch);
};

template <int OB, int AOUT, int AC, bool ACMC, bool BF = false>
KernelSet make_kset() {
  using C = Cfg<OB, AOUT, AC, ACMC, BF>;
  void (*heads)(SacArgs, AcmScratch) = nullptr;
  if constexpr (C::NB_PAIR > 2) heads = k_sac_actor_heads<C>;
  void (*critic)(SacArgs) = k_sac_critic_phase<C>;
#if SPP_BF16_TWO_TILES
  if constexpr (C::BF && C::ACMC && !C::F3) critic = k_sac_critic_phase2<C>;
#endif
  return {critic, k_sac_actor_phase<C>, heads, k_policy_act<C>, k_acm_regress<C>,
          nullptr, nullptr, nullptr, nullptr};
}
template <int OB, int AOUT, int AC, bool ACMC>
KernelSet make_dkset() {
  using D = DCfg<OB, AOUT, AC, ACMC>;
  return {nullptr, nullptr, nullptr, nullptr, nullptr,
          k_ddpg_critic_phase<D>, k_ddpg_actor_phase<D>, k_ddpg_policy_act<D>, k_bacm_regress<D>};
}

#define SPP_KSET_CASE(mk, o, a, c)                                     \
  if (ob == o && aout == a && ac == c) {                               \
    *ks = acmc ? mk<o, a, c, true>() : mk<o, a, c, false>();           \
    return true;                                                       \
  }

bool kset_sac_hopper(int ob, int aout, int ac, bool acmc, KernelSet* ks);
bool kset_sac_hcheetah(int ob, int aout, int ac, bool acmc, KernelSet* ks);
bool kset_sac_ant(int ob, int aout, int ac, bool acmc, KernelSet* ks);
bool kset_sac_small(int ob, int aout, int ac, bool acmc, KernelSet* ks);
bool kset_ddpg(int ob, int aout, int ac, bool acmc, KernelSet* ks);
bool kset_ddpg_ant(int ob, int aout, int ac, bool acmc, KernelSet* ks);
bool kset_sac_bf16(int ob, int aout, int ac, bool acmc, KernelSet* ks);
bool kset_sac_vanilla(int ob, int aout, int ac, bool acmc, KernelSet* ks);
bool kset_ddpg_vanilla(int ob, int aout, int ac, bool acmc, KernelSet* ks);

}
```

### spp-rl_amd/csrc/sac.hip

```cpp
#pragma once
#include "sac_kernels.h"

namespace spp {

constexpr float kLog2 = 0.69314718055994530942f;
constexpr float kLogSqrt2Pi = 0.91893853320467274178f;

template <int OB_, int AOUT_, int AC_, bool ACMC_, bool BF_ = false>
struct Cfg {
  static constexpr int OB = OB_, AOUT = AOUT_, AC = AC_;
  static constexpr bool ACMC = ACMC_;
  static constexpr bool BF = BF_;
  static constexpr bool F3 = !BF_ || SPP_BF16_FUSE3;
  static constexpr int NB_OB = blocks_of(OB);
  static constexpr int NB_AOUT = blocks_of(AOUT);
  static constexpr int NB_H2 = blocks_of(2 * AOUT);
  static constexpr int NB_PAIR = (AOUT + 15) / 16;
  static constexpr int CA = ACMC ? AC : AOUT;
  static constexpr int NB_CA = blocks_of(CA);
  static constexpr int NB_CIN = NB_OB + NB_CA;
  static constexpr int NB_ACMIN = NB_OB + NB_AOUT;
  static constexpr uint64_t RV_X = rv_nat(OB, NB_OB);
  static constexpr uint64_t RV_H = rv_nat(256, 8);
  static constexpr uint64_t RV_CIN = rv_cat(OB, NB_OB, CA, NB_CA);
// ... 296 lines not shown
      }
      setbits(m2lo, m2hi, ob, bits);
    });
  }
  SPP_TP(2);
  {
    dense_lds<NBH, C::BF>(A.Wh, L.img, L.tbl + A.tbh, [&](int ob, const f32x16& acc) {
#pragma unroll
      for (int q = 0; q < 16; ++q) {
        const int ur = 32 * ob + ru(q);
        if (ur + L.h4 < NHR) L.bl[ur * 32] = acc[q];
      }
    });
  }
  SPP_TP(3);
}

template <class C, bool ST>
__device__ __forceinline__ void acm_forward(const SacArgs& p, const f32x16 (&xin)[C::NB_ACMIN], const Lane& L,
                                            float* Z1g, float* Z2g, float* T3g) {
  float* small = L.sl - L.h4 * 32 - L.s;
  const rsrc_t z1r = rsrc(Z1g), z2r = rsrc(Z2g), t3r = rsrc(T3g);
  dense<C::NB_ACMIN, C::RV_ACMIN, C::BF>(p.acm.W1, 2, xin, L.tbl + p.acm.tb1, [&](int ob, const f32x16& acc) {
#pragma unroll
    for (int q = 0; q < 16; ++q) {
      const int ur = 32 * ob + ru(q);
      const float v = tanhf(acc[q]);
      L.sl[ur * 32] = v;
      if constexpr (ST) fm_st(z1r, ur, L.ld4, L.vo, v);
    }
  });
  f32x16 z1[2];
  lds_load<2>(z1, small);
  dense<2, C::RV_Z1, C::BF>(p.acm.W2, 1, z1, L.tbl + p.acm.tb2, [&](int ob, const f32x16& acc) {
#pragma unroll
    for (int q = 0; q < 16; ++q) {
      const float v = tanhf(acc[q]);
      L.sl[ru(q) * 32] = v;
      if constexpr (ST) fm_st(z2r, ru(q), L.ld4, L.vo, v);
    }
  });
  f32x16 z2[1];
  lds_load<1>(z2, small);
  float limv[16];
#pragma unroll
  for (int q = 0; q < 16; ++q) {
    const int u = ru(q) + L.h4;
    limv[q] = acm_lim<true>(p, L.tbl, u < C::AC ? u : 0);
  }
  dense<1, C::RV_Z2, C::BF>(p.acm.W3, 1, z2, L.tbl + p.acm.tb3, [&](int ob, const f32x16& acc) {
#pragma unroll
    for (int q = 0; q < 16; ++q) {
      const int u = ru(q) + L.h4;
      if (u < C::AC) {
        const float t = tanhf(acc[q]);
        L.sl[ru(q) * 32] = t * limv[q];
        if constexpr (ST) fm_st(t3r, ru(q), L.ld4, L.vo, t);
      }
    }
  });
}

template <class C, bool ST, int R = 30, bool H2L = false>
__device__ __forceinline__ float critic_forward(const CriticDev& Q, const f32x16 (&xin)[C::NB_CIN], const Lane& L,
                                                float* H1g, float* H2g, uint64_t& m1lo, uint64_t& m1hi,
                                                uint64_t& m2lo, uint64_t& m2hi) {
  const rsrc_t h1r = rsrc(H1g), h2r = rsrc(H2g);
  float qp = 0.f;
  const float* w3 = L.tbl + Q.tw3;
  auto epi2 = [&](int ob, const f32x16& acc) {
    uint32_t bits = 0;
    float tv[16];
    tvals(w3, ob, L.h4, tv);
#pragma unroll
    for (int q = 0; q < 16; ++q) {
      const float v = fmaxf(acc[q], 0.f);
      if constexpr (H2L) L.bl[(32 * ob + ru(q)) * 32] = v;
      else if constexpr (ST) op_st<C::BF>(h2r, 32 * ob + ru(q), L.ld4, L.vo, v);
      qp = fmaf(v, tv[q], qp);
      bits |= (uint32_t)(v > 0.f) << q;
    }
    setbits(m2lo, m2hi, ob, bits);
  };
  if constexpr (C::GEN_CFC1) {
    const int ld4 = L.ld4;
    const uint32_t vo = L.vo;
    auto st1 = [=](int ur, float v) {
      if constexpr (ST) op_st<C::BF>(h1r, ur, ld4, vo, v);
    };
    Fc1Gen<C::NB_CIN, C::RV_CIN, 8, decltype(st1)> g{xin, rsrc(Q.W1), 16u * lane_id(), L.tbl + Q.tb1, L.h, m1lo, m1hi, st1};
    g.request(0);
    SPP_TP(R);
    dense_gen<8>(Q.W2, L.tbl + Q.tb2, g, epi2);
  } else {
    dense<C::NB_CIN, C::RV_CIN, C::BF>(Q.W1, 8, xin, L.tbl + Q.tb1, [&](int ob, const f32x16& acc) {
      uint32_t bits = 0;
#pragma unroll
      for (int q = 0; q < 16; ++q) {
        const int ur = 32 * ob + ru(q);
        const float v = fmaxf(acc[q], 0.f);
        L.bl[ur * 32] = v;
        if constexpr (ST) op_st<C::BF>(h1r, ur, L.ld4, L.vo, v);
        bits |= (uint32_t)(v > 0.f) << q;
      }
      setbits(m1lo, m1hi, ob, bits);
    });
    SPP_TP(R);
    dense_lds<8, C::BF>(Q.W2, L.img, L.tbl + Q.tb2, epi2);
  }
  SPP_TP(R + 1);
  return qp + __shfl_xor(qp, 32, 64) + *Q.b3;
}

template <class C, bool BRF = false>
__device__ __forceinline__ float squash_write(const SacArgs& p, const f32x16 (&hd)[C::NB_PAIR],
                                              const float* __restrict__ EPS, const Lane& L) {
  float lp = 0.f, corr = 0.f;
  const int h8 = 8 * L.h;
  const rsrc_t er = rsrc_n(EPS, C::AOUT * L.ld4);
  float ev[C::NB_PAIR][8];
#pragma unroll
  for (int ib = 0; ib < C::NB_PAIR; ++ib)
#pragma unroll
    for (int r = 0; r < 8; ++r) ev[ib][r] = 16 * ib + r < C::AOUT ? fm_ldb(er, 16 * ib + r, L.ld4, L.vp) : 0.f;
  constexpr bool kBranchFree = BRF;
#pragma unroll
  for (int ib = 0; ib < C::NB_PAIR; ++ib)
#pragma unroll
    for (int r = 0; r < 8; ++r) {
      const int j0 = 16 * ib + r;
      if (j0 >= C::AOUT) continue;
      const int j = j0 + h8;
      const bool ok = j < C::AOUT;
      if (kBranchFree || ok) {
        const int jj = ok ? j : 0;
        constexpr bool F = C::BF;
        const float mu = hd[ib][r];
        const float ls = fminf(fmaxf(hd[ib][r + 8], -20.f), 2.f);
        const float sc = t_exp<F>(ls);
        const float e = ev[ib][r];
        const float u = fadd_rn(mu, fmul_rn(e, sc));
        float lpj;
        if constexpr (F) {
          lpj = -0.5f * e * e - ls - kLogSqrt2Pi;
        } else {
          const float d = fsub_rn(u, mu);
          const float var = fmul_rn(sc, sc);
          lpj = fsub_rn(fsub_rn(fdiv_rn(-fmul_rn(d, d), 2.f * var), logf(sc)), kLogSqrt2Pi);
        }
        const float cj = 2.f * fsub_rn(fsub_rn(kLog2, u), t_softplus<F>(-2.f * u));
        lp += ok ? lpj : 0.f;
        corr += ok ? cj : 0.f;
        const float a = fmul_rn(t_tanh<F>(u), actor_lim<true>(p, L.tbl, jj));
        const float ad = denorm<true>(p, L.tbl, jj, a);
        if (ok) L.pl[j0 * 32] = ad;
      }
    }
  SPP_XLANE_SYNC();
  const float tot = lp + __shfl_xor(lp, 32, 64);
  const float tc = corr + __shfl_xor(corr, 32, 64);
  return fsub_rn(tot, tc);
}

template <class C>
__global__ __launch_bounds__(256, 1) void k_sac_critic_phase(SacArgs p) {
  __shared__ __attribute__((aligned(16))) float smem[kWavesPerWG * kLdsPerWave];
  __shared__ __attribute__((aligned(16))) float tbl[kTabMax];
  __shared__ __attribute__((aligned(16))) float s_dq[kWavesPerWG][32];
  SPP_TP_INIT();
  load_table(p, tbl);
  const int w = threadIdx.x >> 6, lane = threadIdx.x & 63;
  float* big = smem + w * kLdsPerWave;
  float* small = big + kSmallRow * 32;
  const int ntiles = p.Bp / 32;
  const int ld = p.Bp;
  const float alpha = *p.alpha;
  float w3a[4] = {0.f, 0.f, 0.f, 0.f}, w3b[4] = {0.f, 0.f, 0.f, 0.f}, b3a = 0.f, b3b = 0.f;
  for (int tile = blockIdx.x * kWavesPerWG + w; tile < ntiles; tile += gridDim.x * kWavesPerWG) {
    const Lane L = make_lane(big, small, tbl, ld, tile * 32 + (lane & 31));
    const int b = L.b;
    const bool valid = b < p.B;
    uint64_t d0 = 0, d1 = 0, d2 = 0, d3 = 0;
    SPP_TP(0);
    actor_trunk<C, false>(p.actor, p.S2, C::OB * L.ld4, L, nullptr, nullptr, d0, d1, d2, d3);
    float lp2;
    {
      f32x16 hd[C::NB_PAIR];
      load_pair<C>(hd, big);
      lp2 = squash_write<C, true>(p, hd, p.EPS1, L);
    }
    SPP_TP(4);
    f32x16 tin[C::NB_CIN];
    if constexpr (C::ACMC) {
      f32x16 xin[C::NB_ACMIN];
      load_cat_gl<C::NB_OB, C::NB_AOUT>(xin, p.S2, C::OB * L.ld4, C::OB, L.ld4, L.vo, big, C::AOUT);
      acm_forward<C, false>(p, xin, L, nullptr, nullptr, nullptr);
      load_cat_gl<C::NB_OB, C::NB_CA>(tin, p.S2, C::OB * L.ld4, C::OB, L.ld4, L.vo, small, C::AC);
    } else {
      load_cat_gl<C::NB_OB, C::NB_CA>(tin, p.S2, C::OB * L.ld4, C::OB, L.ld4, L.vo, big, C::AOUT);
    }
    SPP_TP(5);
    const float q1t = critic_forward<C, false, 6>(p.targ[0], tin, L, nullptr, nullptr, d0, d1, d2, d3);
    const float q2t = critic_forward<C, false, 8>(p.targ[1], tin, L, nullptr, nullptr, d0, d1, d2, d3);
    const float notdone = 1.f - p.DN[b];
    const float y = fadd_rn(p.R[b], fmul_rn(p.gamma * notdone, fsub_rn(fminf(q1t, q2t), alpha * lp2)));
    float lq0 = 0.f, lq1 = 0.f;
#pragma unroll 1
    for (int i = 0; i < 2; ++i) {
      uint64_t m1lo = 0, m1hi = 0, m2lo = 0, m2hi = 0;
      f32x16 xin[C::NB_CIN];
      load_cat_gg<C::NB_OB, C::NB_CA>(xin, p.S, C::OB, C::ACMC ? p.AENV : p.ACT, C::CA, L.ld4, L.vo);
      const CriticDev& Q = p.critic[i];
      SPP_TP(10);
      const float q = critic_forward<C, true, 11, C::F3>(Q, xin, L, p.H1[i], C::F3 ? nullptr : p.H2[i], m1lo, m1hi,
                                                        m2lo, m2hi);
      const float diff = fsub_rn(q, y);
      const float dq = valid ? fmul_rn(2.f * diff, p.inv_B) : 0.f;
      const float lqi = (valid && L.h == 0) ? diff * diff : 0.f;
      if (i == 0) lq0 = lqi; else lq1 = lqi;
      if constexpr (!C::F3) {
        if (L.h == 0) p.DQ[i][b] = dq;
      } else {
      if (L.h == 0) s_dq[w][L.s] = dq;
      SPP_XLANE_SYNC();
#pragma unroll
      for (int k = 0; k < 4; ++k) {
        const int u = lane + 64 * k;
        const float* row = big + u * 32;
        float acc = 0.f;
#pragma unroll 8
        for (int j = 0; j < 32; ++j) {
          const int s2 = (j + u) & 31;
          acc = fmaf(row[s2], s_dq[w][s2], acc);
        }
        if (i == 0) w3a[k] += acc;
        else w3b[k] += acc;
      }
      const float dsum = wave_sum(L.h == 0 ? dq : 0.f);
      if (i == 0) b3a += dsum;
      else b3b += dsum;
      SPP_XLANE_SYNC();
      }
      const rsrc_t d2r = rsrc(p.D2[i]);
      const float* w3 = tbl + Q.tw3;
      const rsrc_t d1r = rsrc(p.D1[i]);
      auto epi1 = [&](int ob, const f32x16& acc) {
#pragma unroll
        for (int q2 = 0; q2 < 16; ++q2)
          op_st<C::BF>(d1r, 32 * ob + ru(q2), L.ld4, L.vo, getbit(m1lo, m1hi, ob, q2) ? acc[q2] : 0.f);
      };
      if constexpr (C::GEN_CD2) {
        const int ld4 = L.ld4;
        const uint32_t vo = L.vo;
        auto st2 = [=](int ur, float v) { op_st<C::BF>(d2r, ur, ld4, vo, v); };
        Delta2Gen<8, decltype(st2)> g{w3, L.h4, m2lo, m2hi, dq, st2, {}};
        SPP_TP(13);
        dense_gen<8>(Q.W2T, nullptr, g, epi1);
      } else {
#pragma unroll 1
        for (int ob = 0; ob < 8; ++ob) {
          float tv[16];
          tvals(w3, ob, L.h4, tv);
#pragma unroll
          for (int q2 = 0; q2 < 16; ++q2) {
            const int ur = 32 * ob + ru(q2);
            const float v = getbit(m2lo, m2hi, ob, q2) ? dq * tv[q2] : 0.f;
            L.bl[ur * 32] = v;
            op_st<C::BF>(d2r, ur, L.ld4, L.vo, v);
          }
        }
        SPP_TP(13);
        dense_lds<8, C::BF>(Q.W2T, big, nullptr, epi1);
      }
    }
    SPP_TP(14);
    const float s0 = wave_sum(lq0), s1 = wave_sum(lq1);
    if (lane == 0) {
      p.part[tile * kParts + 0] = s0;
      p.part[tile * kParts + 1] = s1;
    }
    SPP_TP(15);
  }
  if constexpr (C::F3) {
    const int64_t wg = (int64_t)blockIdx.x * kWavesPerWG + w;
    float* o0 = p.W3P[0] + wg * p.w3p_stride;
    float* o1 = p.W3P[1] + wg * p.w3p_stride;
#pragma unroll
    for (int k = 0; k < 4; ++k) {
      o0[lane + 64 * k] = w3a[k];
      o1[lane + 64 * k] = w3b[k];
    }
    if (lane == 0) {
      o0[256] = b3a;
      o1[256] = b3b;
    }
  }
  SPP_TP_FLUSH();
}

struct AcmScratch {
  float *Z1, *Z2, *T3;
  float* GAD;
  uint64_t* MASK;
};

template <class C>
__global__ __launch_bounds__(256, 1) void k_sac_actor_phase(SacArgs p, AcmScratch z) {
  __shared__ float smem[kWavesPerWG * kLdsPerWave];
  __shared__ __attribute__((aligned(16))) float tbl[kTabMax];
  SPP_TP_INIT();
  load_table(p, tbl);
  const int w = threadIdx.x >> 6, lane = threadIdx.x & 63;
  float* big = smem + w * kLdsPerWave;
  float* small = big + kSmallRow * 32;
  const int ntiles = p.Bp / 32;
  const int ld = p.Bp;
  const float alpha = *p.alpha;
  for (int tile = blockIdx.x * kWavesPerWG + w; tile < ntiles; tile += gridDim.x * kWavesPerWG) {
    const Lane L = make_lane(big, small, tbl, ld, tile * 32 + (lane & 31));
    const int b = L.b;
    const bool valid = b < p.B;
    const float g_lp = valid ? alpha * p.inv_B : 0.f;
    uint64_t a1lo = 0, a1hi = 0, a2lo = 0, a2hi = 0;
    SPP_TP(26);
    actor_trunk<C, true>(p.actor, p.S, C::OB * L.ld4, L, p.AH1, p.AH2, a1lo, a1hi, a2lo, a2hi);
    SPP_TP(27);
    f32x16 hd[C::NB_PAIR];
    load_pair<C>(hd, big);
    const float lp = squash_write<C>(p, hd, p.EPS2, L);
    SPP_TP(28);
    constexpr bool kParkHeads = C::NB_PAIR > 2;
    if constexpr (kParkHeads) {
#pragma unroll
      for (int ib = 0; ib < C::NB_PAIR; ++ib)
#pragma unroll
        for (int r = 0; r < 8; ++r) {
          const int j0 = 16 * ib + r;
          if (j0 + 8 * L.h < C::AOUT) {
            fm_st(rsrc(p.ADH), j0, L.ld4, L.vp, hd[ib][r]);
            fm_st(rsrc(p.ADH), C::AOUT + j0, L.ld4, L.vp, hd[ib][r + 8]);
          }
        }
    }
    f32x16 cin[C::NB_CIN];
    if constexpr (C::ACMC) {
      f32x16 xin[C::NB_ACMIN];
      load_cat_gl<C::NB_OB, C::NB_AOUT>(xin, p.S, C::OB * L.ld4, C::OB, L.ld4, L.vo, big, C::AOUT);
      acm_forward<C, true>(p, xin, L, z.Z1, z.Z2, z.T3);
      load_cat_gl<C::NB_OB, C::NB_CA>(cin, p.S, C::OB * L.ld4, C::OB, L.ld4, L.vo, small, C::AC);
    } else {
      load_cat_gl<C::NB_OB, C::NB_CA>(cin, p.S, C::OB * L.ld4, C::OB, L.ld4, L.vo, big, C::AOUT);
    }
    SPP_TP(29);
    uint64_t ma0 = 0, ma1 = 0, ma2 = 0, ma3 = 0, mb0 = 0, mb1 = 0, mb2 = 0, mb3 = 0;
    const float q1 = critic_forward<C, false>(p.critic[0], cin, L, nullptr, nullptr, ma0, ma1, ma2, ma3);
    const float q2 = critic_forward<C, false>(p.critic[1], cin, L, nullptr, nullptr, mb0, mb1, mb2, mb3);
    const float qmin = fminf(q1, q2);
    const float gq = valid ? -p.inv_B : 0.f;
    const float dqa = q1 < q2 ? gq : (q1 == q2 ? 0.5f * gq : 0.f);
    const float dqb = q2 < q1 ? gq : (q1 == q2 ? 0.5f * gq : 0.f);
    SPP_TP(19);
    f32x16 dca[C::NB_CA];
#pragma unroll
    for (int ib = 0; ib < C::NB_CA; ++ib) dca[ib] = zero16();
#pragma unroll 1
    for (int i = 0; i < 2; ++i) {
      const CriticDev& Q = p.critic[i];
      const uint64_t k0 = i ? mb0 : ma0, k1 = i ? mb1 : ma1, k2 = i ? mb2 : ma2, k3 = i ? mb3 : ma3;
      const float dqi = i ? dqb : dqa;
      const float* w3 = tbl + Q.tw3;
      auto epi1 = [&](int ob, const f32x16& acc) {
#pragma unroll
        for (int q = 0; q < 16; ++q) L.bl[(32 * ob + ru(q)) * 32] = getbit(k0, k1, ob, q) ? acc[q] : 0.f;
      };
      if constexpr (C::GEN_AD2) {
        auto st2 = [](int, float) {};
        Delta2Gen<8, decltype(st2)> g{w3, L.h4, k2, k3, dqi, st2, {}};
        SPP_TPN(20);
        dense_gen<8>(Q.W2T, nullptr, g, epi1);
      } else {
#pragma unroll 1
        for (int ob = 0; ob < 8; ++ob) {
          float tv[16];
          tvals(w3, ob, L.h4, tv);
#pragma unroll
          for (int q = 0; q < 16; ++q) L.bl[(32 * ob + ru(q)) * 32] = getbit(k2, k3, ob, q) ? dqi * tv[q] : 0.f;
        }
        SPP_TPN(20);
        dense_lds<8, C::BF>(Q.W2T, big, nullptr, epi1);
      }
      SPP_TPN(21);
      dense_lds<C::NB_CA, C::BF>(Q.W1Ta, big, nullptr, [&](int ob, const f32x16& acc) {
#pragma unroll
        for (int ib = 0; ib < C::NB_CA; ++ib)
          if (ib == ob) dca[ib] += acc;
      });
      SPP_TPN(22);
    }
    SPP_TP(31);
    if constexpr (C::ACMC) {
      constexpr bool kPre = !kParkHeads;
      float t3v[16], limv[16], z2v[16], z1v[2][16];
      const rsrc_t t3r = rsrc_n(z.T3, C::AC * L.ld4);
#pragma unroll
      for (int q = 0; q < 16; ++q) {
        const int u = ru(q) + L.h4;
        t3v[q] = fm_ldb(t3r, ru(q), L.ld4, L.vo);
        limv[q] = acm_lim<true>(p, L.tbl, u < C::AC ? u : 0);
      }
      if constexpr (kPre) {
#pragma unroll
        for (int q = 0; q < 16; ++q) z2v[q] = fm_ld(rsrc(z.Z2), ru(q), L.ld4, L.vo);
#pragma unroll
        for (int ob = 0; ob < 2; ++ob)
#pragma unroll
          for (int q = 0; q < 16; ++q) z1v[ob][q] = fm_ld(rsrc(z.Z1), 32 * ob + ru(q), L.ld4, L.vo);
      }
      auto z2at = [&](int q) {
        if constexpr (kPre) return z2v[q];
        else return fm_ld(rsrc(z.Z2), ru(q), L.ld4, L.vo);
      };
      auto z1at = [&](int ob, int q) {
        if constexpr (kPre) return ob ? z1v[1][q] : z1v[0][q];
        else return fm_ld(rsrc(z.Z1), 32 * ob + ru(q), L.ld4, L.vo);
      };
      f32x16 dp3[1];
#pragma unroll
      for (int q = 0; q < 16; ++q) {
        const int u = ru(q) + L.h4;
        const float t = t3v[q];
        dp3[0][q] = u < C::AC ? dca[0][q] * limv[q] * (1.f - t * t) : 0.f;
      }
      SPP_TPN(23);
      dense<1, C::RV_AC, C::BF>(p.acm.W3T, 1, dp3, nullptr, [&](int ob, const f32x16& acc) {
#pragma unroll
        for (int q = 0; q < 16; ++q) {
          const float zz = z2at(q);
          L.sl[ru(q) * 32] = acc[q] * (1.f - zz * zz);
        }
      });
      SPP_TPN(24);
      f32x16 dp2[1];
      lds_load<1>(dp2, small);
      dense<1, C::RV_Z2, C::BF>(p.acm.W2T, 2, dp2, nullptr, [&](int ob, const f32x16& acc) {
#pragma unroll
        for (int q = 0; q < 16; ++q) {
          const float zz = z1at(ob, q);
          L.sl[(32 * ob + ru(q)) * 32] = acc[q] * (1.f - zz * zz);
        }
      });
      SPP_TPN(25);
      f32x16 dp1[2];
      lds_load<2>(dp1, small);
      dense<2, C::RV_Z1, C::BF>(p.acm.W1Ta, C::NB_AOUT, dp1, nullptr, [&](int ob, const f32x16& acc) {
#pragma unroll
        for (int q = 0; q < 16; ++q) {
          const int ur = 32 * ob + ru(q);
          if (ur + L.h4 < C::AOUT) L.bl[ur * 32] = acc[q];
        }
      });
    } else {
#pragma unroll
      for (int ib = 0; ib < C::NB_CA; ++ib)
#pragma unroll
        for (int q = 0; q < 16; ++q) {
          const int ur = 32 * ib + ru(q);
          if (ur + L.h4 < C::AOUT) L.bl[ur * 32] = dca[ib][q];
        }
    }
    SPP_TP(16);
    if constexpr (kParkHeads) {
      const rsrc_t gr = rsrc(z.GAD);
#pragma unroll
      for (int ib = 0; ib < C::NB_AOUT; ++ib)
#pragma unroll
        for (int q = 0; q < 16; ++q) {
          const int ur = 32 * ib + ru(q);
          if (ur + L.h4 < C::AOUT) fm_st(gr, ur, L.ld4, L.vo, L.bl[ur * 32]);
        }
      uint64_t* mk = z.MASK + (int64_t)tile * 4 * 64 + lane;
      mk[0] = a1lo;
      mk[64] = a1hi;
      mk[128] = a2lo;
      mk[192] = a2hi;
      const float ps = wave_sum((valid && L.h == 0) ? fsub_rn(alpha * lp, qmin) : 0.f);
      const float pl = wave_sum((valid && L.h == 0) ? lp : 0.f);
      if (lane == 0) {
        p.part[tile * kParts + 2] = ps;
        p.part[tile * kParts + 4] = pl;
      }
      continue;
    }
    float sac_part = (valid && L.h == 0) ? fsub_rn(alpha * lp, qmin) : 0.f;
    float dist_part = 0.f;
    const float cl_scale = valid ? p.custom_loss * 2.f * p.inv_B / (float)C::AOUT : 0.f;
    const int h8 = 8 * L.h;
    {
      const rsrc_t adhr = rsrc_n(p.ADH, 2 * C::AOUT * L.ld4);
      const rsrc_t epsr = rsrc_n(p.EPS2, C::AOUT * L.ld4);
      const rsrc_t s2r = rsrc_n(p.S2, C::OB * L.ld4);
      const bool closs = p.custom_loss != 0.f;
      SPP_XLANE_SYNC();
  #pragma unroll
      for (int ib = 0; ib < C::NB_PAIR; ++ib)
  #pragma unroll
        for (int r = 0; r < 8; ++r) {
          const int j0 = 16 * ib + r;
          const int j = j0 + h8;
          const bool ok = j < C::AOUT;
          const int jj = ok ? j : 0;
          const float mu = kParkHeads ? fm_ldb(adhr, j0, L.ld4, L.vp) : hd[ib][r];
          const float lsr = kParkHeads ? fm_ldb(adhr, C::AOUT + j0, L.ld4, L.vp) : hd[ib][r + 8];
          const float e = fm_ldb(epsr, j0, L.ld4, L.vp);
          const float s2 = closs ? fm_ldb(s2r, j0, L.ld4, L.vp) : 0.f;
          const float ls = fminf(fmaxf(lsr, -20.f), 2.f);
          const float sc = expf(ls);
          const float u = fadd_rn(mu, fmul_rn(e, sc));
          const float d = fsub_rn(u, mu);
          const float t = tanhf(u);
          const float lim = actor_lim<true>(p, L.tbl, jj);
          const float a = fmul_rn(t, lim);
          float g_ad = L.pl[j0 * 32];
          float g_a = 0.f;
          if (closs) {
            if (p.norm_closs) {
              const float df = fsub_rn(a, normalize<true>(p, L.tbl, jj, s2));
              g_a += cl_scale * df;
              dist_part += (valid && ok) ? df * df : 0.f;
            } else {
              const float df = fsub_rn(denorm<true>(p, L.tbl, jj, a), s2);
              g_ad += cl_scale * df;
              dist_part += (valid && ok) ? df * df : 0.f;
            }
          }
          g_a += g_ad * denorm_scale<true>(p, L.tbl, jj);
          const float var = fmul_rn(sc, sc);
          const float sig_m2u = 1.f / (1.f + expf(2.f * u));
          const float gu = g_a * lim * (1.f - t * t) + g_lp * (-d / var + 2.f - 4.f * sig_m2u);
          const float gmu = gu + g_lp * d / var;
          const float gsc = gu * e + g_lp * (d * d / (var * sc) - 1.f / sc);
          const float gls = (lsr >= -20.f && lsr <= 2.f) ? gsc * sc : 0.f;
          hd[ib][r] = ok ? gmu : 0.f;
          hd[ib][r + 8] = ok ? gls : 0.f;
        }
  #pragma unroll
      for (int ib = 0; ib < C::NB_PAIR; ++ib)
  #pragma unroll
        for (int r = 0; r < 8; ++r) {
          const int j0 = 16 * ib + r;
          if (j0 + h8 < C::AOUT) {
            fm_st(rsrc(p.ADH), j0, L.ld4, L.vp, hd[ib][r]);
            fm_st(rsrc(p.ADH), C::AOUT + j0, L.ld4, L.vp, hd[ib][r + 8]);
          }
        }
    }
    SPP_TP(17);
    dense<C::NB_PAIR, C::RV_PAIR, C::BF>(p.actor.WhT, 8, hd, nullptr, [&](int ob, const f32x16& acc) {
#pragma unroll
      for (int q = 0; q < 16; ++q) {
        const int ur = 32 * ob + ru(q);
        const float v = getbit(a2lo, a2hi, ob, q) ? acc[q] : 0.f;
        L.bl[ur * 32] = v;
        op_st<C::BF>(rsrc(p.AD2), ur, L.ld4, L.vo, v);
      }
    });
    {
      dense_lds<8, C::BF>(p.actor.W2T, big, nullptr, [&](int ob, const f32x16& acc) {
#pragma unroll
        for (int q = 0; q < 16; ++q)
          op_st<C::BF>(rsrc(p.AD1), 32 * ob + ru(q), L.ld4, L.vo, getbit(a1lo, a1hi, ob, q) ? acc[q] : 0.f);
      });
    }
    SPP_TP(18);
    const float ps = wave_sum(sac_part);
    const float pd = wave_sum(dist_part);
    const float pl = wave_sum((valid && L.h == 0) ? lp : 0.f);
    if (lane == 0) {
      p.part[tile * kParts + 2] = ps;
      p.part[tile * kParts + 3] = pd;
      p.part[tile * kParts + 4] = pl;
    }
  }
  SPP_TP_FLUSH();
}

template <class C>
__global__ __launch_bounds__(256, 1) void k_sac_actor_heads(SacArgs p, AcmScratch z) {
  __shared__ float smem[kWavesPerWG * kLdsPerWave];
  __shared__ __attribute__((aligned(16))) float tbl[kTabMax];
  SPP_TP_INIT();
  load_table(p, tbl);
  const int w = threadIdx.x >> 6, lane = threadIdx.x & 63;
  float* big = smem + w * kLdsPerWave;
  float* small = big + kSmallRow * 32;
  const int ntiles = p.Bp / 32;
  const int ld = p.Bp;
  const float alpha = *p.alpha;
  for (int tile = blockIdx.x * kWavesPerWG + w; tile < ntiles; tile += gridDim.x * kWavesPerWG) {
    const Lane L = make_lane(big, small, tbl, ld, tile * 32 + (lane & 31));
    const bool valid = L.b < p.B;
    const float g_lp = valid ? alpha * p.inv_B : 0.f;
    const uint64_t* mk = z.MASK + (int64_t)tile * 4 * 64 + lane;
    const uint64_t a1lo = mk[0], a1hi = mk[64], a2lo = mk[128], a2hi = mk[192];
    float dist_part = 0.f;
    const float cl_scale = valid ? p.custom_loss * 2.f * p.inv_B / (float)C::AOUT : 0.f;
    const rsrc_t adhr = rsrc_n(p.ADH, 2 * C::AOUT * L.ld4);
    const rsrc_t epsr = rsrc_n(p.EPS2, C::AOUT * L.ld4);
    const rsrc_t s2r = rsrc_n(p.S2, C::OB * L.ld4);
    const rsrc_t gr = rsrc_n(z.GAD, C::AOUT * L.ld4);
    const bool closs = p.custom_loss != 0.f;
    const int h8 = 8 * L.h;
#pragma unroll 1
    for (int ib = 0; ib < C::NB_PAIR; ++ib) {
      float mu[8], lsr[8], ev[8], s2v[8], gv[8];
#pragma unroll
      for (int r = 0; r < 8; ++r) {
        const int j0 = 16 * ib + r;
        mu[r] = fm_ldb(adhr, j0, L.ld4, L.vp);
        lsr[r] = fm_ldb(adhr, C::AOUT + j0, L.ld4, L.vp);
        ev[r] = fm_ldb(epsr, j0, L.ld4, L.vp);
        s2v[r] = closs ? fm_ldb(s2r, j0, L.ld4, L.vp) : 0.f;
        gv[r] = fm_ldb(gr, j0, L.ld4, L.vp);
      }
#pragma unroll
      for (int r = 0; r < 8; ++r) {
        const int j0 = 16 * ib + r;
        const int j = j0 + h8;
        const bool ok = j < C::AOUT;
        const int jj = ok ? j : 0;
        constexpr bool F = C::BF;
        const float e = ev[r];
        const float ls = fminf(fmaxf(lsr[r], -20.f), 2.f);
        const float sc = t_exp<F>(ls);
        const float u = fadd_rn(mu[r], fmul_rn(e, sc));
        const float d = fsub_rn(u, mu[r]);
        const float t = t_tanh<F>(u);
        const float lim = actor_lim<true>(p, L.tbl, jj);
        const float a = fmul_rn(t, lim);
        float g_ad = gv[r];
        float g_a = 0.f;
        if (closs) {
          if (p.norm_closs) {
            const float df = fsub_rn(a, normalize<true>(p, L.tbl, jj, s2v[r]));
            g_a += cl_scale * df;
            dist_part += (valid && ok) ? df * df : 0.f;
          } else {
            const float df = fsub_rn(denorm<true>(p, L.tbl, jj, a), s2v[r]);
            g_ad += cl_scale * df;
            dist_part += (valid && ok) ? df * df : 0.f;
          }
        }
        g_a += g_ad * denorm_scale<true>(p, L.tbl, jj);
        const float var = fmul_rn(sc, sc);
        const float ivar = t_rcp<F>(var), isc = t_rcp<F>(sc);
        const float sig_m2u = t_rcp<F>(1.f + t_exp<F>(2.f * u));
        const float gu = g_a * lim * (1.f - t * t) + g_lp * (-d * ivar + 2.f - 4.f * sig_m2u);
        const float gmu = gu + g_lp * d * ivar;
        const float gsc = gu * e + g_lp * (d * d * ivar * isc - isc);
        const float gls = (lsr[r] >= -20.f && lsr[r] <= 2.f) ? gsc * sc : 0.f;
        if (ok) {
          L.pl[j0 * 32] = gmu;
          L.pl[(C::AOUT + j0) * 32] = gls;
        }
      }
    }
    f32x16 hd[C::NB_PAIR];
    load_pair<C>(hd, big);
#pragma unroll
    for (int ib = 0; ib < C::NB_PAIR; ++ib)
#pragma unroll
      for (int r = 0; r < 8; ++r) {
        const int j0 = 16 * ib + r;
        if (j0 + h8 < C::AOUT) {
          fm_st(rsrc(p.ADH), j0, L.ld4, L.vp, hd[ib][r]);
          fm_st(rsrc(p.ADH), C::AOUT + j0, L.ld4, L.vp, hd[ib][r + 8]);
        }
      }
    SPP_TP(17);
    dense<C::NB_PAIR, C::RV_PAIR, C::BF>(p.actor.WhT, 8, hd, nullptr, [&](int ob, const f32x16& acc) {
#pragma unroll
      for (int q = 0; q < 16; ++q) {
        const int ur = 32 * ob + ru(q);
        const float v = getbit(a2lo, a2hi, ob, q) ? acc[q] : 0.f;
        L.bl[ur * 32] = v;
        op_st<C::BF>(rsrc(p.AD2), ur, L.ld4, L.vo, v);
      }
    });
    dense_lds<8, C::BF>(p.actor.W2T, big, nullptr, [&](int ob, const f32x16& acc) {
#pragma unroll
      for (int q = 0; q < 16; ++q)
        op_st<C::BF>(rsrc(p.AD1), 32 * ob + ru(q), L.ld4, L.vo, getbit(a1lo, a1hi, ob, q) ? acc[q] : 0.f);
    });
    SPP_TP(18);
    const float pd = wave_sum(dist_part);
    if (lane == 0) p.part[tile * kParts + 3] = pd;
  }
  SPP_TP_FLUSH();
}

struct ActArgs {
  int E, mode, denorm_out;
  float act_noise;
  const float *obs, *eps, *noise;
  float *target_out, *env_out;
  int plain;
};

template <class C>
__global__ __launch_bounds__(256, 1) void k_policy_act(SacArgs p, ActArgs a) {
  __shared__ float smem[kWavesPerWG * kLdsPerWave];
  __shared__ __attribute__((aligned(16))) float tbl[kTabMax];
  load_table(p, tbl);
  const int w = threadIdx.x >> 6, lane = threadIdx.x & 63;
  float* big = smem + w * kLdsPerWave;
  float* small = big + kSmallRow * 32;
  const int ntiles = (a.E + 31) / 32;
  for (int tile = blockIdx.x * kWavesPerWG + w; tile < ntiles; tile += gridDim.x * kWavesPerWG) {
    const int e = tile * 32 + (lane & 31);
    const bool valid = e < a.E;
    const int er = valid ? e : 0;
    Lane L = make_lane(big, small, tbl, 1, er * C::OB);
    const bool use_actor = a.mode == 1 || a.mode == 2;
    if (use_actor) {
      uint64_t d0 = 0, d1 = 0, d2 = 0, d3 = 0;
      actor_trunk<C, false>(p.actor, a.obs, a.E * C::OB * 4, L, nullptr, nullptr, d0, d1, d2, d3);
    }
    f32x16 hd[C::NB_PAIR];
    if (use_actor) load_pair<C>(hd, big);
    const int h8 = 8 * L.h;
#pragma unroll
    for (int ib = 0; ib < C::NB_PAIR; ++ib)
#pragma unroll
      for (int r = 0; r < 8; ++r) {
        const int j0 = 16 * ib + r;
        const int j = j0 + h8;
        if (j < C::AOUT) {
          const float lim = actor_lim<true>(p, L.tbl, j);
          float act;
          if (a.plain && (a.mode == 0 || a.mode == 3)) {
            act = valid ? a.eps[er * C::AOUT + j] : 0.f;
          } else if (a.plain) {
            const float mu = hd[ib][r];
            float u = mu;
            if (a.mode == 1 && a.eps) {
              const float ls = fminf(fmaxf(hd[ib][r + 8], -20.f), 2.f);
              u = fadd_rn(mu, fmul_rn(valid ? a.eps[er * C::AOUT + j] : 0.f, expf(ls)));
            }
            act = fmul_rn(tanhf(u), lim);
            if (a.mode == 1 && a.noise) act = fadd_rn(act, a.act_noise * (valid ? a.noise[er * C::AOUT + j] : 0.f));
            act = fminf(fmaxf(act, -lim), lim);
          } else if (a.mode == 0) {
            act = valid ? lim * a.eps[er * C::AOUT + j] : 0.f;
          } else if (a.mode == 3) {
            act = valid ? a.eps[er * C::AOUT + j] : 0.f;
          } else {
            const float mu = hd[ib][r];
            float u = mu;
            if (a.mode == 1 && a.eps) {
              const float ls = fminf(fmaxf(hd[ib][r + 8], -20.f), 2.f);
              u = fadd_rn(mu, fmul_rn(valid ? a.eps[er * C::AOUT + j] : 0.f, expf(ls)));
            }
            act = fmul_rn(tanhf(u), lim);
            if (a.mode == 1 && a.noise) act += fmul_rn(a.act_noise * (valid ? a.noise[er * C::AOUT + j] : 0.f), lim);
            act = fminf(fmaxf(act, -1.1f * lim), 1.1f * lim);
          }
          if (a.denorm_out && !a.plain) act = denorm<true>(p, L.tbl, j, act);
          L.pl[j0 * 32] = act;
          if (valid) a.target_out[er * C::AOUT + j] = act;
          if (valid && a.plain) a.env_out[er * C::AOUT + j] = act;
        }
      }
    if (a.plain) continue;
    f32x16 xin[C::NB_ACMIN];
    load_cat_gl<C::NB_OB, C::NB_AOUT>(xin, a.obs, a.E * C::OB * 4, C::OB, L.ld4, L.vo, big, C::AOUT);
    acm_forward<C, false>(p, xin, L, nullptr, nullptr, nullptr);
    if (L.h == 0 && valid)
      for (int u = 0; u < C::AC; ++u) a.env_out[er * C::AC + u] = small[u * 32 + L.s];
  }
}

struct AcmRegArgs {
  int B, Bp;
  const float *x, *y;
  float *XT, *Z1, *Z2, *P1, *P2, *P3;
  float* part;
};

template <class C>
__global__ __launch_bounds__(256, 1) void k_acm_regress(SacArgs p, AcmRegArgs g) {
  __shared__ float smem[kWavesPerWG * kLdsPerWave];
  __shared__ __attribute__((aligned(16))) float tbl[kTabMax];
  load_table(p, tbl);
  const int w = threadIdx.x >> 6, lane = threadIdx.x & 63;
  float* big = smem + w * kLdsPerWave;
  float* small = big + kSmallRow * 32;
  const int ntiles = g.Bp / 32;
  const int ld = g.Bp;
  constexpr int IN = 2 * C::OB;
  constexpr int NB_IN = blocks_of(IN);
  constexpr uint64_t RV_IN = rv_nat(IN, NB_IN);
  for (int tile = blockIdx.x * kWavesPerWG + w; tile < ntiles; tile += gridDim.x * kWavesPerWG) {
    const Lane L = make_lane(big, small, tbl, ld, tile * 32 + (lane & 31));
    const int b = L.b;
    const bool valid = b < g.B;
    const int br = valid ? b : 0;
    f32x16 xin[NB_IN];
#pragma unroll
    for (int ib = 0; ib < NB_IN; ++ib)
#pragma unroll
      for (int r = 0; r < 16; ++r) {
        const int ur = 32 * ib + ru(r);
        const int u = ur + L.h4;
        xin[ib][r] = (u < IN && valid) ? g.x[br * IN + u] : 0.f;
      }
#pragma unroll
    for (int ib = 0; ib < NB_IN; ++ib)
#pragma unroll
      for (int r = 0; r < 16; ++r) {
        const int ur = 32 * ib + ru(r);
        if (ur + L.h4 < IN) fm_st(rsrc(g.XT), ur, L.ld4, L.vo, xin[ib][r]);
      }
    dense<NB_IN, RV_IN, C::BF>(p.acm.W1, 2, xin, tbl + p.acm.tb1, [&](int ob, const f32x16& acc) {
#pragma unroll
      for (int q = 0; q < 16; ++q) {
        const int ur = 32 * ob + ru(q);
        const float v = tanhf(acc[q]);
        L.sl[ur * 32] = v;
        fm_st(rsrc(g.Z1), ur, L.ld4, L.vo, v);
      }
    });
    f32x16 z1[2];
    lds_load<2>(z1, small);
    dense<2, C::RV_Z1, C::BF>(p.acm.W2, 1, z1, tbl + p.acm.tb2, [&](int ob, const f32x16& acc) {
#pragma unroll
      for (int q = 0; q < 16; ++q) {
        const float v = tanhf(acc[q]);
        L.sl[ru(q) * 32] = v;
        fm_st(rsrc(g.Z2), ru(q), L.ld4, L.vo, v);
      }
    });
    f32x16 z2[1];
    lds_load<1>(z2, small);
    float lsum = 0.f;
    f32x16 p3[1];
    const float sc = 2.f / ((float)g.B * (float)C::AC);
    float limv[16], yv[16];
#pragma unroll
    for (int q = 0; q < 16; ++q) {
      const int u = ru(q) + L.h4;
      const int uu = u < C::AC ? u : 0;
      limv[q] = acm_lim<true>(p, L.tbl, uu);
      yv[q] = g.y[br * C::AC + uu];
    }
    dense<1, C::RV_Z2, C::BF>(p.acm.W3, 1, z2, tbl + p.acm.tb3, [&](int ob, const f32x16& acc) {
#pragma unroll
      for (int q = 0; q < 16; ++q) {
        const int u = ru(q) + L.h4;
        float v = 0.f;
        if (u < C::AC && valid) {
          const float t = tanhf(acc[q]);
          const float lim = limv[q];
          const float df = fsub_rn(fmul_rn(t, lim), yv[q]);
          lsum += df * df;
          v = sc * df * lim * (1.f - t * t);
        }
        p3[0][q] = v;
        if (u < C::AC) fm_st(rsrc(g.P3), ru(q), L.ld4, L.vo, v);
      }
    });
    dense<1, C::RV_AC, C::BF>(p.acm.W3T, 1, p3, nullptr, [&](int ob, const f32x16& acc) {
#pragma unroll
      for (int q = 0; q < 16; ++q) {
        const float zz = z2[0][q];
        const float v = acc[q] * (1.f - zz * zz);
        L.sl[ru(q) * 32] = v;
        fm_st(rsrc(g.P2), ru(q), L.ld4, L.vo, v);
      }
    });
    f32x16 p2[1];
    lds_load<1>(p2, small);
    dense<1, C::RV_Z2, C::BF>(p.acm.W2T, 2, p2, nullptr, [&](int ob, const f32x16& acc) {
#pragma unroll
      for (int q = 0; q < 16; ++q) {
        const int ur = 32 * ob + ru(q);
        const float zz = ob == 0 ? z1[0][q] : z1[1][q];
        fm_st(rsrc(g.P1), ur, L.ld4, L.vo, acc[q] * (1.f - zz * zz));
      }
    });
    const float ls = wave_sum(lsum);
    if (lane == 0) g.part[tile] = ls;
  }
}

#ifndef SPP_KSET_TU
struct StageArgs {
  int B, Bp, ob, aout, ac;
  const float *obs, *next_obs, *act, *rew, *acm;
  const int8_t* done;
  const float *eps1, *eps2;
  float *S, *S2, *ACT, *AENV, *R, *DN, *EPS1, *EPS2;
};
__global__ void k_stage_batch(StageArgs a) {
  const int64_t b = (int64_t)blockIdx.x * blockDim.x + threadIdx.x;
  if (b >= a.Bp) return;
  const bool v = b < a.B;
  const int64_t ld = a.Bp;
  for (int f = 0; f < a.ob; ++f) {
    a.S[f * ld + b] = v ? a.obs[b * a.ob + f] : 0.f;
    a.S2[f * ld + b] = v ? a.next_obs[b * a.ob + f] : 0.f;
  }
  for (int f = 0; f < a.aout; ++f) {
    if (a.act) a.ACT[f * ld + b] = v ? a.act[b * a.aout + f] : 0.f;
    if (a.eps1) a.EPS1[f * ld + b] = v ? a.eps1[b * a.aout + f] : 0.f;
    if (a.eps2) a.EPS2[f * ld + b] = v ? a.eps2[b * a.aout + f] : 0.f;
  }
  for (int f = 0; f < a.ac; ++f) a.AENV[f * ld + b] = v ? a.acm[b * a.ac + f] : 0.f;
  a.R[b] = v ? a.rew[b] : 0.f;
  a.DN[b] = v ? (float)a.done[b] : 0.f;
}

__global__ void k_eps_copy_fm(const float* eps, float* E, int aout, int B, int Bp) {
  const int64_t i = (int64_t)blockIdx.x * blockDim.x + threadIdx.x;
  if (i >= (int64_t)aout * Bp) return;
  const int64_t j = i / Bp, b = i % Bp;
  E[i] = b < B ? eps[b * aout + j] : 0.f;
}

__global__ void k_eps_read_fm(const float* E, float* eps, int aout, int B, int Bp) {
  const int64_t i = (int64_t)blockIdx.x * blockDim.x + threadIdx.x;
  if (i >= (int64_t)aout * B) return;
  const int64_t b = i / aout, j = i % aout;
  eps[i] = E[j * Bp + b];
}

__device__ __forceinline__ void box_muller_hw(uint32_t a, uint32_t b, float& n0, float& n1) {
  const float u = u01(a), v = u01(b);
  const float r = __builtin_amdgcn_sqrtf(-2.f * 0.69314718055994531f * __builtin_amdgcn_logf(u));
  n0 = r * __builtin_amdgcn_cosf(v);
  n1 = r * __builtin_amdgcn_sinf(v);
}
__global__ void k_eps_fm(float* E, int aout, int B, int Bp, uint64_t seed, uint64_t ctr, float* E2, uint64_t ctr2) {
  if (blockIdx.y) {
    E = E2;
    ctr = ctr2;
  }
  const int i = blockIdx.x * blockDim.x + threadIdx.x;
  if (4 * i >= aout * Bp) return;
  const u32x4 r = philox(seed, ctr, (uint64_t)i);
  float4 v;
  box_muller_hw(r.x, r.y, v.x, v.y);
  box_muller_hw(r.z, r.w, v.z, v.w);
  const int col = (4 * i) % Bp;
  v.x = col < B ? v.x : 0.f;
  v.y = col + 1 < B ? v.y : 0.f;
  v.z = col + 2 < B ? v.z : 0.f;
  v.w = col + 3 < B ? v.w : 0.f;
  *reinterpret_cast<float4*>(E + 4 * (int64_t)i) = v;
}

#endif

template <int NBI, int NBO, int KQ = 0>
__global__ __launch_bounds__(64) void k_debug_dense(const float4* Wf, const float* bias, const float* x, float* y,
                                                    int B, int K, int N, int act) {
  __shared__ float img[256 * 32];
  __shared__ __attribute__((aligned(16))) float tb[256];
  const int lane = threadIdx.x & 63, h = lane >> 5, s = lane & 31;
  for (int i = lane; i < 256; i += 64) tb[i] = (bias && i < N) ? bias[i] : 0.f;
  const int64_t b = (int64_t)blockIdx.x * 32 + s;
  f32x16 in[NBI];
#pragma unroll
  for (int ib = 0; ib < NBI; ++ib)
#pragma unroll
    for (int r = 0; r < 16; ++r) {
      const int u = 32 * ib + unit_of(r, h);
      in[ib][r] = (u < K && b < B) ? x[b * K + u] : 0.f;
      img[(32 * ib + ru(r) + 4 * h) * 32 + s] = in[ib][r];
    }
  __syncthreads();
  auto epi = [&](int ob, const f32x16& acc) {
#pragma unroll
    for (int q = 0; q < 16; ++q) {
      const int u = 32 * ob + unit_of(q, h);
      float v = acc[q];
      if (act == 1) v = fmaxf(v, 0.f);
      if (act == 2) v = tanhf(v);
      if (u < N && b < B) y[b * N + u] = v;
    }
  };
  if constexpr (NBI == 8)
    dense_lds<NBO>(Wf, img, tb, epi);
  else
    dense<NBI, KQ ? (uint64_t)KQ : rv_nat(32 * NBI, NBI)>(Wf, (N + 31) / 32, in, tb, epi);
}

}
```

Measured before the change: 431,800.

## Split SAC actor phase to backprop only through the min-Q critic per sample

Splits the fused actor kernel into forward, min-Q backward, and heads-backward kernels. A scan and scatter build compacted per-critic sample lists, so the critic backward runs only for the critic that attains the minimum (both on ties) instead of for both critics on every sample. This roughly halves critic backward work, at the cost of extra launches, scratch traffic for masks and dCA, and gather-indexed memory access. It is on by default for non-team fp32 configurations and can be disabled with SPP_MINQ_SPLIT=0.

```diff
diff --git a/spp-rl_amd/csrc/api.hip b/spp-rl_amd/csrc/api.hip
--- a/spp-rl_amd/csrc/api.hip
+++ b/spp-rl_amd/csrc/api.hip
@@ -833,6 +833,8 @@
   float *aux = nullptr;
   float* GAD = nullptr;
   uint64_t* MASK = nullptr;
+  bool minq_split = false;
+  AcmScratch mq{};
   float *RX = nullptr, *RZ1 = nullptr, *RZ2 = nullptr, *RP1 = nullptr, *RP2 = nullptr, *RP3 = nullptr;
   DwSet dws[2];
   DevArray<AdamJob> d_adam;
@@ -1381,6 +1383,8 @@
   {
     const char* t = getenv("SPP_SAC_TEAM");
     a->team_ok = !(t && t[0] == '0');
+    const char* m = getenv("SPP_MINQ_SPLIT");
+    a->minq_split = ks.actor_fwd && ks.actor_minq && ks.actor_bwd && !(m && m[0] == '0');
   }
   const int ob = cfg->ob, aout = cfg->aout, ac = cfg->ac;
   a->cin = ob + (cfg->acm_critic ? ac : aout);
@@ -1413,6 +1417,10 @@
                 oRP2 = take(dd ? 64 : 32), oRP3 = take(ac);
   const int64_t oRS21 = dd ? take(64) : 0, oRPZ21 = dd ? take(64) : 0;
   const int64_t oGAD = take(aout), oMASK = take(16);
+  const bool mq = a->minq_split;
+  const int64_t ca = a->cin - ob;
+  const int64_t oSEL = mq ? take(1) : 0, oCM = mq ? take(32) : 0, oCNT = mq ? take(1) : 0, oLIST = mq ? take(2) : 0,
+                oDCA = mq ? take(2 * ca) : 0;
   const int64_t oPart = total;
   total += ntiles * kBParts + 64;
   const int64_t oAux = total;
@@ -1433,6 +1441,19 @@
   a->Z1 = b + oZ1; a->Z2 = b + oZ2; a->T3 = b + oT3;
   a->GAD = b + oGAD;
   a->MASK = reinterpret_cast<uint64_t*>(b + oMASK);
+  if (mq) {
+    AcmScratch& q = a->mq;
+    q.Z1 = a->Z1; q.Z2 = a->Z2; q.T3 = a->T3; q.GAD = a->GAD; q.MASK = a->MASK;
+    q.SEL = reinterpret_cast<uint8_t*>(b + oSEL);
+    q.CM = reinterpret_cast<uint64_t*>(b + oCM);
+    q.CNT = reinterpret_cast<uint32_t*>(b + oCNT);
+    q.OFF = q.CNT + ntiles;
+    q.NG = reinterpret_cast<int*>(q.OFF + 2 * ntiles);
+    q.LIST[0] = reinterpret_cast<int*>(b + oLIST);
+    q.LIST[1] = q.LIST[0] + Bp;
+    q.DCA[0] = b + oDCA;
+    q.DCA[1] = q.DCA[0] + ca * Bp;
+  }
   a->RX = b + oRX; a->RZ1 = b + oRZ1; a->RZ2 = b + oRZ2; a->RP1 = b + oRP1; a->RP2 = b + oRP2; a->RP3 = b + oRP3;
   if (dd) {
     a->bz = BAcmScratch{a->Z1, a->Z2, a->T3};
@@ -1598,8 +1619,18 @@
   const int grid = sac_grid(a, p.Bp);
   tmark(a, 1, st);
   const bool team = sac_team(a, p.Bp);
-  hipLaunchKernelGGL(team ? a->ks.actor_team : a->ks.actor, dim3(grid), dim3(team ? 64 * kTeamActor : 256), 0, st, p, z);
-  if (a->ks.actor_heads) hipLaunchKernelGGL(a->ks.actor_heads, dim3(grid), dim3(256), 0, st, p, z);
+  if (!team && a->minq_split) {
+    z = a->mq;
+    hipLaunchKernelGGL(a->ks.actor_fwd, dim3(grid), dim3(256), 0, st, p, z);
+    hipLaunchKernelGGL(k_minq_scan, dim3(1), dim3(kMinqScanThreads), 0, st, (const uint32_t*)z.CNT, z.OFF, z.NG, p.Bp / 32);
+    hipLaunchKernelGGL(k_minq_scatter, dim3(cdiv(p.Bp, 256)), dim3(256), 0, st, (const uint8_t*)z.SEL,
+                       (const uint32_t*)z.OFF, z.LIST[0], z.LIST[1], p.Bp);
+    hipLaunchKernelGGL(a->ks.actor_minq, dim3(grid), dim3(256), 0, st, p, z);
+    hipLaunchKernelGGL(a->ks.actor_bwd, dim3(grid), dim3(256), 0, st, p, z);
+  } else {
+    hipLaunchKernelGGL(team ? a->ks.actor_team : a->ks.actor, dim3(grid), dim3(team ? 64 * kTeamActor : 256), 0, st, p, z);
+    if (a->ks.actor_heads) hipLaunchKernelGGL(a->ks.actor_heads, dim3(grid), dim3(256), 0, st, p, z);
+  }
   tmark(a, 1, st);
   SPP_CHECK_HIP(hipGetLastError());
   tmark(a, 2, st);
diff --git a/spp-rl_amd/csrc/kset.h b/spp-rl_amd/csrc/kset.h
--- a/spp-rl_amd/csrc/kset.h
+++ b/spp-rl_amd/csrc/kset.h
@@ -23,6 +23,9 @@
   void (*dcritic_team)(SacArgs, BAcmScratch);
   void (*dactor_team)(SacArgs, BAcmScratch);
   void (*dact_team)(SacArgs, ActArgs, BAcmScratch);
+  void (*actor_fwd)(SacArgs, AcmScratch);
+  void (*actor_minq)(SacArgs, AcmScratch);
+  void (*actor_bwd)(SacArgs, AcmScratch);
 };
 
 template <int OB, int AOUT, int AC, bool ACMC, bool BF = false>
@@ -34,8 +37,14 @@
 #if SPP_BF16_TWO_TILES
   if constexpr (C::BF && C::ACMC && !C::F3) critic = k_sac_critic_phase2<C>;
 #endif
-  return {critic, k_sac_actor_phase<C>, heads, k_policy_act<C>, k_acm_regress<C>,
-          nullptr, nullptr, nullptr, nullptr};
+  KernelSet ks{critic, k_sac_actor_phase<C>, heads, k_policy_act<C>, k_acm_regress<C>,
+               nullptr, nullptr, nullptr, nullptr};
+  if constexpr (!C::BF) {
+    ks.actor_fwd = k_sac_actor_phase<C, true>;
+    ks.actor_minq = k_sac_minq_backward<C>;
+    ks.actor_bwd = k_sac_actor_heads<C, true>;
+  }
+  return ks;
 }
 template <int OB, int AOUT, int AC, bool ACMC>
 KernelSet make_dkset() {
diff --git a/spp-rl_amd/csrc/sac.hip b/spp-rl_amd/csrc/sac.hip
--- a/spp-rl_amd/csrc/sac.hip
+++ b/spp-rl_amd/csrc/sac.hip
@@ -622,9 +622,164 @@
   float *Z1, *Z2, *T3;
   float* GAD;
   uint64_t* MASK;
+  uint8_t* SEL;
+  uint64_t* CM;
+  uint32_t *CNT, *OFF;
+  int* NG;
+  int* LIST[2];
+  float* DCA[2];
 };
 
-template <class C>
+template <class C, bool PRE>
+__device__ __forceinline__ void acm_backward(const SacArgs& p, const AcmScratch& z, const Lane& L, float* small,
+                                             const f32x16 (&dca)[C::NB_CA]) {
+  constexpr bool kPre = PRE;
+  float t3v[16], limv[16], z2v[16], z1v[2][16];
+  const rsrc_t t3r = rsrc_n(z.T3, C::AC * L.ld4);
+#pragma unroll
+  for (int q = 0; q < 16; ++q) {
+    const int u = ru(q) + L.h4;
+    t3v[q] = fm_ldb(t3r, ru(q), L.ld4, L.vo);
+    limv[q] = acm_lim<true>(p, L.tbl, u < C::AC ? u : 0);
+  }
+  if constexpr (kPre) {
+#pragma unroll
+    for (int q = 0; q < 16; ++q) z2v[q] = fm_ld(rsrc(z.Z2), ru(q), L.ld4, L.vo);
+#pragma unroll
+    for (int ob = 0; ob < 2; ++ob)
+#pragma unroll
+      for (int q = 0; q < 16; ++q) z1v[ob][q] = fm_ld(rsrc(z.Z1), 32 * ob + ru(q), L.ld4, L.vo);
+  }
+  auto z2at = [&](int q) {
+    if constexpr (kPre) return z2v[q];
+    else return fm_ld(rsrc(z.Z2), ru(q), L.ld4, L.vo);
+  };
+  auto z1at = [&](int ob, int q) {
+    if constexpr (kPre) return ob ? z1v[1][q] : z1v[0][q];
+    else return fm_ld(rsrc(z.Z1), 32 * ob + ru(q), L.ld4, L.vo);
+  };
+  f32x16 dp3[1];
+#pragma unroll
+  for (int q = 0; q < 16; ++q) {
+    const int u = ru(q) + L.h4;
+    const float t = t3v[q];
+    dp3[0][q] = u < C::AC ? dca[0][q] * limv[q] * (1.f - t * t) : 0.f;
+  }
+  SPP_TPN(23);
+  dense<1, C::RV_AC, C::BF>(p.acm.W3T, 1, dp3, nullptr, [&](int ob, const f32x16& acc) {
+#pragma unroll
+    for (int q = 0; q < 16; ++q) {
+      const float zz = z2at(q);
+      L.sl[ru(q) * 32] = acc[q] * (1.f - zz * zz);
+    }
+  });
+  SPP_TPN(24);
+  f32x16 dp2[1];
+  lds_load<1>(dp2, small);
+  dense<1, C::RV_Z2, C::BF>(p.acm.W2T, 2, dp2, nullptr, [&](int ob, const f32x16& acc) {
+#pragma unroll
+    for (int q = 0; q < 16; ++q) {
+      const float zz = z1at(ob, q);
+      L.sl[(32 * ob + ru(q)) * 32] = acc[q] * (1.f - zz * zz);
+    }
+  });
+  SPP_TPN(25);
+  f32x16 dp1[2];
+  lds_load<2>(dp1, small);
+  dense<2, C::RV_Z1, C::BF>(p.acm.W1Ta, C::NB_AOUT, dp1, nullptr, [&](int ob, const f32x16& acc) {
+#pragma unroll
+    for (int q = 0; q < 16; ++q) {
+      const int ur = 32 * ob + ru(q);
+      if (ur + L.h4 < C::AOUT) L.bl[ur * 32] = acc[q];
+    }
+  });
+}
+template <class C, bool PRE>
+__device__ __forceinline__ void dca_to_dad(const SacArgs& p, const AcmScratch& z, const Lane& L, float* small,
+                                           const f32x16 (&dca)[C::NB_CA]) {
+  if constexpr (C::ACMC) {
+    acm_backward<C, PRE>(p, z, L, small, dca);
+  } else {
+#pragma unroll
+    for (int ib = 0; ib < C::NB_CA; ++ib)
+#pragma unroll
+      for (int q = 0; q < 16; ++q) {
+        const int ur = 32 * ib + ru(q);
+        if (ur + L.h4 < C::AOUT) L.bl[ur * 32] = dca[ib][q];
+      }
+  }
+}
+
+template <class C, bool PARK>
+__device__ __forceinline__ float heads_backward(const SacArgs& p, const Lane& L, f32x16 (&hd)[C::NB_PAIR], bool valid,
+                                                float g_lp) {
+  constexpr bool kParkHeads = PARK;
+  float dist_part = 0.f;
+  const float cl_scale = valid ? p.custom_loss * 2.f * p.inv_B / (float)C::AOUT : 0.f;
+  const int h8 = 8 * L.h;
+  {
+    const rsrc_t adhr = rsrc_n(p.ADH, 2 * C::AOUT * L.ld4);
+    const rsrc_t epsr = rsrc_n(p.EPS2, C::AOUT * L.ld4);
+    const rsrc_t s2r = rsrc_n(p.S2, C::OB * L.ld4);
+    const bool closs = p.custom_loss != 0.f;
+    SPP_XLANE_SYNC();
+#pragma unroll
+    for (int ib = 0; ib < C::NB_PAIR; ++ib)
+#pragma unroll
+      for (int r = 0; r < 8; ++r) {
+        const int j0 = 16 * ib + r;
+        const int j = j0 + h8;
+        const bool ok = j < C::AOUT;
+        const int jj = ok ? j : 0;
+        const float mu = kParkHeads ? fm_ldb(adhr, j0, L.ld4, L.vp) : hd[ib][r];
+        const float lsr = kParkHeads ? fm_ldb(adhr, C::AOUT + j0, L.ld4, L.vp) : hd[ib][r + 8];
+        const float e = fm_ldb(epsr, j0, L.ld4, L.vp);
+        const float s2 = closs ? fm_ldb(s2r, j0, L.ld4, L.vp) : 0.f;
+        const float ls = fminf(fmaxf(lsr, -20.f), 2.f);
+        const float sc = expf(ls);
+        const float u = fadd_rn(mu, fmul_rn(e, sc));
+        const float d = fsub_rn(u, mu);
+        const float t = tanhf(u);
+        const float lim = actor_lim<true>(p, L.tbl, jj);
+        const float a = fmul_rn(t, lim);
+        float g_ad = L.pl[j0 * 32];
+        float g_a = 0.f;
+        if (closs) {
+          if (p.norm_closs) {
+            const float df = fsub_rn(a, normalize<true>(p, L.tbl, jj, s2));
+            g_a += cl_scale * df;
+            dist_part += (valid && ok) ? df * df : 0.f;
+          } else {
+            const float df = fsub_rn(denorm<true>(p, L.tbl, jj, a), s2);
+            g_ad += cl_scale * df;
+            dist_part += (valid && ok) ? df * df : 0.f;
+          }
+        }
+        g_a += g_ad * denorm_scale<true>(p, L.tbl, jj);
+        const float var = fmul_rn(sc, sc);
+        const float sig_m2u = 1.f / (1.f + expf(2.f * u));
+        const float gu = g_a * lim * (1.f - t * t) + g_lp * (-d / var + 2.f - 4.f * sig_m2u);
+        const float gmu = gu + g_lp * d / var;
+        const float gsc = gu * e + g_lp * (d * d / (var * sc) - 1.f / sc);
+        const float gls = (lsr >= -20.f && lsr <= 2.f) ? gsc * sc : 0.f;
+        hd[ib][r] = ok ? gmu : 0.f;
+        hd[ib][r + 8] = ok ? gls : 0.f;
+      }
+#pragma unroll
+    for (int ib = 0; ib < C::NB_PAIR; ++ib)
+#pragma unroll
+      for (int r = 0; r < 8; ++r) {
+        const int j0 = 16 * ib + r;
+        if (j0 + h8 < C::AOUT) {
+          fm_st(rsrc(p.ADH), j0, L.ld4, L.vp, hd[ib][r]);
+          fm_st(rsrc(p.ADH), C::AOUT + j0, L.ld4, L.vp, hd[ib][r + 8]);
+        }
+      }
+  }
+  return dist_part;
+}
+
+template <class C, bool SPLIT = false>
 __global__ __launch_bounds__(256, 1) void k_sac_actor_phase(SacArgs p, AcmScratch z) {
   __shared__ float smem[kWavesPerWG * kLdsPerWave];
   __shared__ __attribute__((aligned(16))) float tbl[kTabMax];
@@ -649,7 +804,8 @@
     load_pair<C>(hd, big);
     const float lp = squash_write<C>(p, hd, p.EPS2, L);
     SPP_TP(28);
-    constexpr bool kParkHeads = C::NB_PAIR > 2;
+    constexpr bool kWide = C::NB_PAIR > 2;
+    constexpr bool kParkHeads = kWide || SPLIT;
     if constexpr (kParkHeads) {
 #pragma unroll
       for (int ib = 0; ib < C::NB_PAIR; ++ib)
@@ -680,6 +836,30 @@
     const float dqa = q1 < q2 ? gq : (q1 == q2 ? 0.5f * gq : 0.f);
     const float dqb = q2 < q1 ? gq : (q1 == q2 ? 0.5f * gq : 0.f);
     SPP_TP(19);
+    if constexpr (SPLIT) {
+      const int sel = valid ? (int)(q1 <= q2) | ((int)(q2 <= q1) << 1) : 0;
+      if (L.h == 0) z.SEL[b] = (uint8_t)sel;
+      uint4* cm0 = reinterpret_cast<uint4*>(z.CM + ((int64_t)b * 2 + L.h) * 4);
+      uint4* cm1 = reinterpret_cast<uint4*>(z.CM + (((int64_t)ld + b) * 2 + L.h) * 4);
+      cm0[0] = make_uint4((uint32_t)ma0, (uint32_t)(ma0 >> 32), (uint32_t)ma1, (uint32_t)(ma1 >> 32));
+      cm0[1] = make_uint4((uint32_t)ma2, (uint32_t)(ma2 >> 32), (uint32_t)ma3, (uint32_t)(ma3 >> 32));
+      cm1[0] = make_uint4((uint32_t)mb0, (uint32_t)(mb0 >> 32), (uint32_t)mb1, (uint32_t)(mb1 >> 32));
+      cm1[1] = make_uint4((uint32_t)mb2, (uint32_t)(mb2 >> 32), (uint32_t)mb3, (uint32_t)(mb3 >> 32));
+      const int n1 = __popcll(__ballot(L.h == 0 && (sel & 1))), n2 = __popcll(__ballot(L.h == 0 && (sel & 2)));
+      uint64_t* mk = z.MASK + (int64_t)tile * 4 * 64 + lane;
+      mk[0] = a1lo;
+      mk[64] = a1hi;
+      mk[128] = a2lo;
+      mk[192] = a2hi;
+      const float ps = wave_sum((valid && L.h == 0) ? fsub_rn(alpha * lp, qmin) : 0.f);
+      const float pl = wave_sum((valid && L.h == 0) ? lp : 0.f);
+      if (lane == 0) {
+        z.CNT[tile] = (uint32_t)n1 | ((uint32_t)n2 << 16);
+        p.part[tile * kParts + 2] = ps;
+        p.part[tile * kParts + 4] = pl;
+      }
+      continue;
+    }
     f32x16 dca[C::NB_CA];
 #pragma unroll
     for (int ib = 0; ib < C::NB_CA; ++ib) dca[ib] = zero16();
@@ -718,78 +898,9 @@
       SPP_TPN(22);
     }
     SPP_TP(31);
-    if constexpr (C::ACMC) {
-      constexpr bool kPre = !kParkHeads;
-      float t3v[16], limv[16], z2v[16], z1v[2][16];
-      const rsrc_t t3r = rsrc_n(z.T3, C::AC * L.ld4);
-#pragma unroll
-      for (int q = 0; q < 16; ++q) {
-        const int u = ru(q) + L.h4;
-        t3v[q] = fm_ldb(t3r, ru(q), L.ld4, L.vo);
-        limv[q] = acm_lim<true>(p, L.tbl, u < C::AC ? u : 0);
-      }
-      if constexpr (kPre) {
-#pragma unroll
-        for (int q = 0; q < 16; ++q) z2v[q] = fm_ld(rsrc(z.Z2), ru(q), L.ld4, L.vo);
-#pragma unroll
-        for (int ob = 0; ob < 2; ++ob)
-#pragma unroll
-          for (int q = 0; q < 16; ++q) z1v[ob][q] = fm_ld(rsrc(z.Z1), 32 * ob + ru(q), L.ld4, L.vo);
-      }
-      auto z2at = [&](int q) {
-        if constexpr (kPre) return z2v[q];
-        else return fm_ld(rsrc(z.Z2), ru(q), L.ld4, L.vo);
-      };
-      auto z1at = [&](int ob, int q) {
-        if constexpr (kPre) return ob ? z1v[1][q] : z1v[0][q];
-        else return fm_ld(rsrc(z.Z1), 32 * ob + ru(q), L.ld4, L.vo);
-      };
-      f32x16 dp3[1];
-#pragma unroll
-      for (int q = 0; q < 16; ++q) {
-        const int u = ru(q) + L.h4;
-        const float t = t3v[q];
-        dp3[0][q] = u < C::AC ? dca[0][q] * limv[q] * (1.f - t * t) : 0.f;
-      }
-      SPP_TPN(23);
-      dense<1, C::RV_AC, C::BF>(p.acm.W3T, 1, dp3, nullptr, [&](int ob, const f32x16& acc) {
-#pragma unroll
-        for (int q = 0; q < 16; ++q) {
-          const float zz = z2at(q);
-          L.sl[ru(q) * 32] = acc[q] * (1.f - zz * zz);
-        }
-      });
-      SPP_TPN(24);
-      f32x16 dp2[1];
-      lds_load<1>(dp2, small);
-      dense<1, C::RV_Z2, C::BF>(p.acm.W2T, 2, dp2, nullptr, [&](int ob, const f32x16& acc) {
-#pragma unroll
-        for (int q = 0; q < 16; ++q) {
-          const float zz = z1at(ob, q);
-          L.sl[(32 * ob + ru(q)) * 32] = acc[q] * (1.f - zz * zz);
-        }
-      });
-      SPP_TPN(25);
-      f32x16 dp1[2];
-      lds_load<2>(dp1, small);
-      dense<2, C::RV_Z1, C::BF>(p.acm.W1Ta, C::NB_AOUT, dp1, nullptr, [&](int ob, const f32x16& acc) {
-#pragma unroll
-        for (int q = 0; q < 16; ++q) {
-          const int ur = 32 * ob + ru(q);
-          if (ur + L.h4 < C::AOUT) L.bl[ur * 32] = acc[q];
-        }
-      });
-    } else {
-#pragma unroll
-      for (int ib = 0; ib < C::NB_CA; ++ib)
-#pragma unroll
-        for (int q = 0; q < 16; ++q) {
-          const int ur = 32 * ib + ru(q);
-          if (ur + L.h4 < C::AOUT) L.bl[ur * 32] = dca[ib][q];
-        }
-    }
+    dca_to_dad<C, !kWide>(p, z, L, small, dca);
     SPP_TP(16);
-    if constexpr (kParkHeads) {
+    if constexpr (kWide) {
       const rsrc_t gr = rsrc(z.GAD);
 #pragma unroll
       for (int ib = 0; ib < C::NB_AOUT; ++ib)
@@ -812,68 +923,7 @@
       continue;
     }
     float sac_part = (valid && L.h == 0) ? fsub_rn(alpha * lp, qmin) : 0.f;
-    float dist_part = 0.f;
-    const float cl_scale = valid ? p.custom_loss * 2.f * p.inv_B / (float)C::AOUT : 0.f;
-    const int h8 = 8 * L.h;
-    {
-      const rsrc_t adhr = rsrc_n(p.ADH, 2 * C::AOUT * L.ld4);
-      const rsrc_t epsr = rsrc_n(p.EPS2, C::AOUT * L.ld4);
-      const rsrc_t s2r = rsrc_n(p.S2, C::OB * L.ld4);
-      const bool closs = p.custom_loss != 0.f;
-      SPP_XLANE_SYNC();
-  #pragma unroll
-      for (int ib = 0; ib < C::NB_PAIR; ++ib)
-  #pragma unroll
-        for (int r = 0; r < 8; ++r) {
-          const int j0 = 16 * ib + r;
-          const int j = j0 + h8;
-          const bool ok = j < C::AOUT;
-          const int jj = ok ? j : 0;
-          const float mu = kParkHeads ? fm_ldb(adhr, j0, L.ld4, L.vp) : hd[ib][r];
-          const float lsr = kParkHeads ? fm_ldb(adhr, C::AOUT + j0, L.ld4, L.vp) : hd[ib][r + 8];
-          const float e = fm_ldb(epsr, j0, L.ld4, L.vp);
-          const float s2 = closs ? fm_ldb(s2r, j0, L.ld4, L.vp) : 0.f;
-          const float ls = fminf(fmaxf(lsr, -20.f), 2.f);
-          const float sc = expf(ls);
-          const float u = fadd_rn(mu, fmul_rn(e, sc));
-          const float d = fsub_rn(u, mu);
-          const float t = tanhf(u);
-          const float lim = actor_lim<true>(p, L.tbl, jj);
-          const float a = fmul_rn(t, lim);
-          float g_ad = L.pl[j0 * 32];
-          float g_a = 0.f;
-          if (closs) {
-            if (p.norm_closs) {
-              const float df = fsub_rn(a, normalize<true>(p, L.tbl, jj, s2));
-              g_a += cl_scale * df;
-              dist_part += (valid && ok) ? df * df : 0.f;
-            } else {
-              const float df = fsub_rn(denorm<true>(p, L.tbl, jj, a), s2);
-              g_ad += cl_scale * df;
-              dist_part += (valid && ok) ? df * df : 0.f;
-            }
-          }
-          g_a += g_ad * denorm_scale<true>(p, L.tbl, jj);
-          const float var = fmul_rn(sc, sc);
-          const float sig_m2u = 1.f / (1.f + expf(2.f * u));
-          const float gu = g_a * lim * (1.f - t * t) + g_lp * (-d / var + 2.f - 4.f * sig_m2u);
-          const float gmu = gu + g_lp * d / var;
-          const float gsc = gu * e + g_lp * (d * d / (var * sc) - 1.f / sc);
-          const float gls = (lsr >= -20.f && lsr <= 2.f) ? gsc * sc : 0.f;
-          hd[ib][r] = ok ? gmu : 0.f;
-          hd[ib][r + 8] = ok ? gls : 0.f;
-        }
-  #pragma unroll
-      for (int ib = 0; ib < C::NB_PAIR; ++ib)
-  #pragma unroll
-        for (int r = 0; r < 8; ++r) {
-          const int j0 = 16 * ib + r;
-          if (j0 + h8 < C::AOUT) {
-            fm_st(rsrc(p.ADH), j0, L.ld4, L.vp, hd[ib][r]);
-            fm_st(rsrc(p.ADH), C::AOUT + j0, L.ld4, L.vp, hd[ib][r + 8]);
-          }
-        }
-    }
+    const float dist_part = heads_backward<C, false>(p, L, hd, valid, g_lp);
     SPP_TP(17);
     dense<C::NB_PAIR, C::RV_PAIR, C::BF>(p.actor.WhT, 8, hd, nullptr, [&](int ob, const f32x16& acc) {
 #pragma unroll
@@ -904,7 +954,88 @@
   SPP_TP_FLUSH();
 }
 
-template <class C>
+template <class C, bool IMG>
+__device__ __forceinline__ float heads_backward_wide(const SacArgs& p, const AcmScratch& z, const Lane& L,
+                                                     f32x16 (&hd)[C::NB_PAIR], bool valid, float g_lp) {
+  float dist_part = 0.f;
+  const float cl_scale = valid ? p.custom_loss * 2.f * p.inv_B / (float)C::AOUT : 0.f;
+  const rsrc_t adhr = rsrc_n(p.ADH, 2 * C::AOUT * L.ld4);
+  const rsrc_t epsr = rsrc_n(p.EPS2, C::AOUT * L.ld4);
+  const rsrc_t s2r = rsrc_n(p.S2, C::OB * L.ld4);
+  const rsrc_t gr = rsrc_n(z.GAD, C::AOUT * L.ld4);
+  const bool closs = p.custom_loss != 0.f;
+  const int h8 = 8 * L.h;
+  if constexpr (IMG) SPP_XLANE_SYNC();
+#pragma unroll 1
+  for (int ib = 0; ib < C::NB_PAIR; ++ib) {
+    float mu[8], lsr[8], ev[8], s2v[8], gv[8];
+#pragma unroll
+    for (int r = 0; r < 8; ++r) {
+      const int j0 = 16 * ib + r;
+      mu[r] = fm_ldb(adhr, j0, L.ld4, L.vp);
+      lsr[r] = fm_ldb(adhr, C::AOUT + j0, L.ld4, L.vp);
+      ev[r] = fm_ldb(epsr, j0, L.ld4, L.vp);
+      s2v[r] = closs ? fm_ldb(s2r, j0, L.ld4, L.vp) : 0.f;
+      if constexpr (IMG) gv[r] = j0 + h8 < C::AOUT ? L.pl[j0 * 32] : 0.f;
+      else gv[r] = fm_ldb(gr, j0, L.ld4, L.vp);
+    }
+#pragma unroll
+    for (int r = 0; r < 8; ++r) {
+      const int j0 = 16 * ib + r;
+      const int j = j0 + h8;
+      const bool ok = j < C::AOUT;
+      const int jj = ok ? j : 0;
+      constexpr bool F = C::BF;
+      const float e = ev[r];
+      const float ls = fminf(fmaxf(lsr[r], -20.f), 2.f);
+      const float sc = t_exp<F>(ls);
+      const float u = fadd_rn(mu[r], fmul_rn(e, sc));
+      const float d = fsub_rn(u, mu[r]);
+      const float t = t_tanh<F>(u);
+      const float lim = actor_lim<true>(p, L.tbl, jj);
+      const float a = fmul_rn(t, lim);
+      float g_ad = gv[r];
+      float g_a = 0.f;
+      if (closs) {
+        if (p.norm_closs) {
+          const float df = fsub_rn(a, normalize<true>(p, L.tbl, jj, s2v[r]));
+          g_a += cl_scale * df;
+          dist_part += (valid && ok) ? df * df : 0.f;
+        } else {
+          const float df = fsub_rn(denorm<true>(p, L.tbl, jj, a), s2v[r]);
+          g_ad += cl_scale * df;
+          dist_part += (valid && ok) ? df * df : 0.f;
+        }
+      }
+      g_a += g_ad * denorm_scale<true>(p, L.tbl, jj);
+      const float var = fmul_rn(sc, sc);
+      const float ivar = t_rcp<F>(var), isc = t_rcp<F>(sc);
+      const float sig_m2u = t_rcp<F>(1.f + t_exp<F>(2.f * u));
+      const float gu = g_a * lim * (1.f - t * t) + g_lp * (-d * ivar + 2.f - 4.f * sig_m2u);
+      const float gmu = gu + g_lp * d * ivar;
+      const float gsc = gu * e + g_lp * (d * d * ivar * isc - isc);
+      const float gls = (lsr[r] >= -20.f && lsr[r] <= 2.f) ? gsc * sc : 0.f;
+      if (ok) {
+        L.pl[j0 * 32] = gmu;
+        L.pl[(C::AOUT + j0) * 32] = gls;
+      }
+    }
+  }
+  load_pair<C>(hd, L.img);
+#pragma unroll
+  for (int ib = 0; ib < C::NB_PAIR; ++ib)
+#pragma unroll
+    for (int r = 0; r < 8; ++r) {
+      const int j0 = 16 * ib + r;
+      if (j0 + h8 < C::AOUT) {
+        fm_st(rsrc(p.ADH), j0, L.ld4, L.vp, hd[ib][r]);
+        fm_st(rsrc(p.ADH), C::AOUT + j0, L.ld4, L.vp, hd[ib][r + 8]);
+      }
+    }
+  return dist_part;
+}
+
+template <class C, bool SPLIT = false>
 __global__ __launch_bounds__(256, 1) void k_sac_actor_heads(SacArgs p, AcmScratch z) {
   __shared__ float smem[kWavesPerWG * kLdsPerWave];
   __shared__ __attribute__((aligned(16))) float tbl[kTabMax];
@@ -920,82 +1051,38 @@
     const Lane L = make_lane(big, small, tbl, ld, tile * 32 + (lane & 31));
     const bool valid = L.b < p.B;
     const float g_lp = valid ? alpha * p.inv_B : 0.f;
+    constexpr bool kWide = C::NB_PAIR > 2;
+    if constexpr (SPLIT) {
+      const int sel = z.SEL[L.b];
+      const rsrc_t r1 = rsrc_n(z.DCA[0], C::CA * L.ld4), r2 = rsrc_n(z.DCA[1], C::CA * L.ld4);
+      f32x16 dca[C::NB_CA];
+#pragma unroll
+      for (int ib = 0; ib < C::NB_CA; ++ib)
+#pragma unroll
+        for (int q = 0; q < 16; ++q) {
+          const int ur = 32 * ib + ru(q);
+          float v1 = 0.f, v2 = 0.f;
+          if (ur < C::CA) {
+            v1 = fm_ldb(r1, ur, L.ld4, L.vo);
+            v2 = fm_ldb(r2, ur, L.ld4, L.vo);
+          }
+          v1 = (sel & 1) ? v1 : 0.f;
+          v2 = (sel & 2) ? v2 : 0.f;
+          dca[ib][q] = fadd_rn(fadd_rn(0.f, v1), v2);
+        }
+      SPP_TP(31);
+      dca_to_dad<C, true>(p, z, L, small, dca);
+      SPP_TP(16);
+    }
     const uint64_t* mk = z.MASK + (int64_t)tile * 4 * 64 + lane;
     const uint64_t a1lo = mk[0], a1hi = mk[64], a2lo = mk[128], a2hi = mk[192];
     float dist_part = 0.f;
-    const float cl_scale = valid ? p.custom_loss * 2.f * p.inv_B / (float)C::AOUT : 0.f;
-    const rsrc_t adhr = rsrc_n(p.ADH, 2 * C::AOUT * L.ld4);
-    const rsrc_t epsr = rsrc_n(p.EPS2, C::AOUT * L.ld4);
-    const rsrc_t s2r = rsrc_n(p.S2, C::OB * L.ld4);
-    const rsrc_t gr = rsrc_n(z.GAD, C::AOUT * L.ld4);
-    const bool closs = p.custom_loss != 0.f;
-    const int h8 = 8 * L.h;
-#pragma unroll 1
-    for (int ib = 0; ib < C::NB_PAIR; ++ib) {
-      float mu[8], lsr[8], ev[8], s2v[8], gv[8];
-#pragma unroll
-      for (int r = 0; r < 8; ++r) {
-        const int j0 = 16 * ib + r;
-        mu[r] = fm_ldb(adhr, j0, L.ld4, L.vp);
-        lsr[r] = fm_ldb(adhr, C::AOUT + j0, L.ld4, L.vp);
-        ev[r] = fm_ldb(epsr, j0, L.ld4, L.vp);
-        s2v[r] = closs ? fm_ldb(s2r, j0, L.ld4, L.vp) : 0.f;
-        gv[r] = fm_ldb(gr, j0, L.ld4, L.vp);
-      }
-#pragma unroll
-      for (int r = 0; r < 8; ++r) {
-        const int j0 = 16 * ib + r;
-        const int j = j0 + h8;
-        const bool ok = j < C::AOUT;
-        const int jj = ok ? j : 0;
-        constexpr bool F = C::BF;
-        const float e = ev[r];
-        const float ls = fminf(fmaxf(lsr[r], -20.f), 2.f);
-        const float sc = t_exp<F>(ls);
-        const float u = fadd_rn(mu[r], fmul_rn(e, sc));
-        const float d = fsub_rn(u, mu[r]);
-        const float t = t_tanh<F>(u);
-        const float lim = actor_lim<true>(p, L.tbl, jj);
-        const float a = fmul_rn(t, lim);
-        float g_ad = gv[r];
-        float g_a = 0.f;
-        if (closs) {
-          if (p.norm_closs) {
-            const float df = fsub_rn(a, normalize<true>(p, L.tbl, jj, s2v[r]));
-            g_a += cl_scale * df;
-            dist_part += (valid && ok) ? df * df : 0.f;
-          } else {
-            const float df = fsub_rn(denorm<true>(p, L.tbl, jj, a), s2v[r]);
-            g_ad += cl_scale * df;
-            dist_part += (valid && ok) ? df * df : 0.f;
-          }
-        }
-        g_a += g_ad * denorm_scale<true>(p, L.tbl, jj);
-        const float var = fmul_rn(sc, sc);
-        const float ivar = t_rcp<F>(var), isc = t_rcp<F>(sc);
-        const float sig_m2u = t_rcp<F>(1.f + t_exp<F>(2.f * u));
-        const float gu = g_a * lim * (1.f - t * t) + g_lp * (-d * ivar + 2.f - 4.f * sig_m2u);
-        const float gmu = gu + g_lp * d * ivar;
-        const float gsc = gu * e + g_lp * (d * d * ivar * isc - isc);
-        const float gls = (lsr[r] >= -20.f && lsr[r] <= 2.f) ? gsc * sc : 0.f;
-        if (ok) {
-          L.pl[j0 * 32] = gmu;
-          L.pl[(C::AOUT + j0) * 32] = gls;
-        }
-      }
-    }
     f32x16 hd[C::NB_PAIR];
-    load_pair<C>(hd, big);
-#pragma unroll
-    for (int ib = 0; ib < C::NB_PAIR; ++ib)
-#pragma unroll
-      for (int r = 0; r < 8; ++r) {
-        const int j0 = 16 * ib + r;
-        if (j0 + h8 < C::AOUT) {
-          fm_st(rsrc(p.ADH), j0, L.ld4, L.vp, hd[ib][r]);
-          fm_st(rsrc(p.ADH), C::AOUT + j0, L.ld4, L.vp, hd[ib][r + 8]);
-        }
-      }
+    if constexpr (!kWide) {
+      dist_part = heads_backward<C, true>(p, L, hd, valid, g_lp);
+    } else {
+      dist_part = heads_backward_wide<C, SPLIT>(p, z, L, hd, valid, g_lp);
+    }
     SPP_TP(17);
     dense<C::NB_PAIR, C::RV_PAIR, C::BF>(p.actor.WhT, 8, hd, nullptr, [&](int ob, const f32x16& acc) {
 #pragma unroll
@@ -1017,6 +1104,118 @@
   }
   SPP_TP_FLUSH();
 }
+
+template <class C>
+__global__ __launch_bounds__(256, 1) void k_sac_minq_backward(SacArgs p, AcmScratch z) {
+  __shared__ float smem[kWavesPerWG * kLdsPerWave];
+  __shared__ __attribute__((aligned(16))) float tbl[kTabMax];
+  SPP_TP_INIT();
+  load_table(p, tbl);
+  const int w = __builtin_amdgcn_readfirstlane(threadIdx.x >> 6), lane = threadIdx.x & 63;
+  float* big = smem + w * kLdsPerWave;
+  float* small = big + kSmallRow * 32;
+  const int ld = p.Bp;
+  const int n1 = z.NG[0], n2 = z.NG[1];
+  const int g1 = (n1 + 31) >> 5, ngroups = g1 + ((n2 + 31) >> 5);
+  for (int g = blockIdx.x * kWavesPerWG + w; g < ngroups; g += gridDim.x * kWavesPerWG) {
+    const int i = g >= g1;
+    const int pos = 32 * (i ? g - g1 : g) + (lane & 31);
+    const bool live = pos < (i ? n2 : n1);
+    const int b = live ? z.LIST[i][pos] : 0;
+    const Lane L = make_lane(big, small, tbl, ld, b);
+    const uint4* cm = reinterpret_cast<const uint4*>(z.CM + (((int64_t)i * ld + b) * 2 + L.h) * 4);
+    const uint4 c01 = cm[0], c23 = cm[1];
+    const int sel = z.SEL[b];
+    const uint64_t k0 = live ? (uint64_t)c01.x | ((uint64_t)c01.y << 32) : 0;
+    const uint64_t k1 = live ? (uint64_t)c01.z | ((uint64_t)c01.w << 32) : 0;
+    const uint64_t k2 = live ? (uint64_t)c23.x | ((uint64_t)c23.y << 32) : 0;
+    const uint64_t k3 = live ? (uint64_t)c23.z | ((uint64_t)c23.w << 32) : 0;
+    const float gq = -p.inv_B;
+    const float dqi = live ? (sel == 3 ? 0.5f * gq : gq) : 0.f;
+    const CriticDev& Q = p.critic[i];
+    const float* w3 = tbl + Q.tw3;
+    auto epi1 = [&](int ob, const f32x16& acc) {
+#pragma unroll
+      for (int q = 0; q < 16; ++q) L.bl[(32 * ob + ru(q)) * 32] = getbit(k0, k1, ob, q) ? acc[q] : 0.f;
+    };
+    if constexpr (C::GEN_AD2) {
+      auto st2 = [](int, float) {};
+      Delta2Gen<8, decltype(st2)> gen{w3, L.h4, k2, k3, dqi, st2, {}};
+      SPP_TPN(20);
+      dense_gen<8>(Q.W2T, nullptr, gen, epi1);
+    } else {
+#pragma unroll 1
+      for (int ob = 0; ob < 8; ++ob) {
+        float tv[16];
+        tvals(w3, ob, L.h4, tv);
+#pragma unroll
+        for (int q = 0; q < 16; ++q) L.bl[(32 * ob + ru(q)) * 32] = getbit(k2, k3, ob, q) ? dqi * tv[q] : 0.f;
+      }
+      SPP_TPN(20);
+      dense_lds<8, C::BF>(Q.W2T, big, nullptr, epi1);
+    }
+    SPP_TPN(21);
+    const rsrc_t dr = rsrc(z.DCA[i]);
+    dense_lds<C::NB_CA, C::BF>(Q.W1Ta, big, nullptr, [&](int ob, const f32x16& acc) {
+#pragma unroll
+      for (int q = 0; q < 16; ++q) {
+        const int ur = 32 * ob + ru(q);
+        if (ur < C::CA) {
+          if (live && ur + L.h4 < C::CA) fm_st(dr, ur, L.ld4, L.vo, acc[q]);
+        }
+      }
+    });
+    SPP_TPN(22);
+  }
+  SPP_TP_FLUSH();
+}
+
+#ifndef SPP_KSET_TU
+constexpr int kMinqScanThreads = 1024;
+__global__ __launch_bounds__(kMinqScanThreads) void k_minq_scan(const uint32_t* CNT, uint32_t* OFF, int* NG, int ntiles) {
+  __shared__ uint32_t s1[kMinqScanThreads], s2[kMinqScanThreads];
+  const int t = threadIdx.x;
+  const int per = (ntiles + kMinqScanThreads - 1) / kMinqScanThreads;
+  const int t0 = min(t * per, ntiles), t1 = min(t0 + per, ntiles);
+  uint32_t a1 = 0, a2 = 0;
+  for (int k = t0; k < t1; ++k) {
+    const uint32_t c = CNT[k];
+    a1 += c & 0xffffu;
+    a2 += c >> 16;
+  }
+  s1[t] = a1;
+  s2[t] = a2;
+  __syncthreads();
+  for (int o = 1; o < kMinqScanThreads; o <<= 1) {
+    const uint32_t u1 = t >= o ? s1[t - o] : 0u, u2 = t >= o ? s2[t - o] : 0u;
+    __syncthreads();
+    s1[t] += u1;
+    s2[t] += u2;
+    __syncthreads();
+  }
+  uint32_t o1 = s1[t] - a1, o2 = s2[t] - a2;
+  for (int k = t0; k < t1; ++k) {
+    const uint32_t c = CNT[k];
+    OFF[2 * k] = o1;
+    OFF[2 * k + 1] = o2;
+    o1 += c & 0xffffu;
+    o2 += c >> 16;
+  }
+  if (t == kMinqScanThreads - 1) {
+    NG[0] = (int)s1[t];
+    NG[1] = (int)s2[t];
+  }
+}
+__global__ __launch_bounds__(256) void k_minq_scatter(const uint8_t* SEL, const uint32_t* OFF, int* L1, int* L2, int Bp) {
+  const int b = blockIdx.x * blockDim.x + threadIdx.x;
+  const int sel = b < Bp ? SEL[b] : 0;
+  const int sh = threadIdx.x & 32;
+  const uint32_t below = (1u << (threadIdx.x & 31)) - 1u;
+  const uint32_t m1 = (uint32_t)(__ballot(sel & 1) >> sh), m2 = (uint32_t)(__ballot(sel & 2) >> sh);
+  if (sel & 1) L1[OFF[2 * (b >> 5)] + __popc(m1 & below)] = b;
+  if (sel & 2) L2[OFF[2 * (b >> 5) + 1] + __popc(m2 & below)] = b;
+}
+#endif
 
 struct ActArgs {
   int E, mode, denorm_out;
```

After: 453,400 (median of 6 runs). 5.0% higher.
